# zerr0o/whisper-burn

Measured on AMD Instinct MI355X. Metric: real-time factor (audio-s/wall-s) Whisper Large-V3 Q4 @1/2/4/8 MI355X, higher is better.
Workload: dtype fp16x2

## Files before the change

### include/whisper_amd.h

```cpp
#ifndef WHISPER_AMD_H
#define WHISPER_AMD_H

#include <stddef.h>
#include <stdint.h>

#include "wq4.h"

#ifdef __cplusplus
extern "C" {
#endif

typedef struct wa_model wa_model;

typedef enum wa_variant { WA_LARGE_V3 = 0, WA_MEDIUM = 1, WA_TINY_TEST = 2 } wa_variant;

enum {
  WA_CFG_N_MELS = 0,
  WA_CFG_N_AUDIO_CTX,
  WA_CFG_N_AUDIO_STATE,
  WA_CFG_N_AUDIO_HEAD,
  WA_CFG_N_AUDIO_LAYER,
  WA_CFG_N_TEXT_CTX,
  WA_CFG_N_TEXT_STATE,
  WA_CFG_N_TEXT_HEAD,
  WA_CFG_N_TEXT_LAYER,
  WA_CFG_N_VOCAB,
  WA_CFG_N_LANG,
  WA_CFG_COUNT
};

const char* wa_last_error(void);

wq4_status wa_model_create_synthetic(int device, int variant, uint64_t seed, int max_batch, wq4_precision prec,
                                     wa_model** out);
wq4_status wa_model_create_synthetic_ex(int device, int variant, uint64_t seed, int max_batch, wq4_precision prec,
                                        int weight_type, wa_model** out);
int wa_model_weight_type(const wa_model* m);
int wa_model_wide_range(const wa_model* m);
wq4_status wa_model_create_from_gguf(int device, const char* path, int variant, int max_batch, wq4_precision prec,
                                     wa_model** out);
void wa_model_destroy(wa_model* m);

typedef struct wa_gguf wa_gguf;
wq4_status wa_gguf_open(const char* path, wa_gguf** out);
void wa_gguf_close(wa_gguf* g);
int wa_gguf_version(const wa_gguf* g);
int64_t wa_gguf_tensor_count(const wa_gguf* g);
wq4_status wa_gguf_tensor_info(const wa_gguf* g, int64_t index, char* name, size_t name_cap, int* ndims,
                               uint64_t* dims, int* type, uint64_t* offset, uint64_t* nbytes);
wq4_status wa_gguf_tensor_data(const wa_gguf* g, const char* name, uint8_t* out, size_t cap);
wq4_status wa_model_config(const wa_model* m, int32_t* cfg );
size_t wa_model_device_bytes(const wa_model* m);

wq4_status wa_transcribe(wa_model* m, const float* mel_dev, int n_clips, int lang_token, int max_tokens,
                         int eot_stop, int32_t* tokens_out, int32_t* n_tokens_out, void* stream);

wq4_status wa_transcribe_batches(wa_model* m, const float* mel_dev, int n_batches, int n_clips, int lang_token,
                                 int max_tokens, int eot_stop, int32_t* tokens_out, int32_t* n_tokens_out,
                                 void* stream);
wq4_status wa_last_pipeline_stats(const wa_model* m, float* out );
int wa_last_pipeline_pairs(const wa_model* m);

wq4_status wa_log_mel(int device, const float* audio_dev, int n_clips, int64_t n_samples, int64_t ld_audio,
                      int n_mels, float* mel_dev, void* stream);
wq4_status wa_mel_filterbank(int n_mels, float* filters_out, float* window_out);

wq4_status wa_last_timings(const wa_model* m, float* out );

#define WA_PROF_CATEGORIES 4
wq4_status wa_profile_enable(wa_model* m, int enable);
wq4_status wa_profile_read(wa_model* m, double* out , int reset);

#define WA_PROBE_OUT 6
wq4_status wa_probe_kernels(wa_model* m, int n_clips, int iters, double* out, int out_len);
int wa_decode_group_rows(int n_clips);

wq4_status wa_encode(wa_model* m, const float* mel_dev, int n_clips, float* enc_out_dev, void* stream);
wq4_status wa_prompt_logits(wa_model* m, const int32_t* prompt_dev, int n_clips, int plen, float* logits_dev,
                            void* stream);
wq4_status wa_xattn_check(int device, const float* q_dev, const uint8_t* wk_dev, const uint8_t* wv_dev,
                          const float* bv_dev, int weight_type, const float* enc_dev, int n_clips, int Tq, int T,
                          int H, wq4_precision prec, float* out_dev);
wq4_status wa_xattn_kv_check(int device, const float* q_dev, const float* k_dev, const float* v_dev, int n_clips,
                             int Tq, int T, int H, wq4_precision prec, float* out_dev);

wq4_status wa_transcribe_trace(wa_model* m, const float* mel_dev, int n_clips, int lang_token, int max_tokens,
                               int eot_stop, int32_t* tokens_out, int32_t* n_tokens_out, const int32_t* trace_ids_dev,
                               int trace_k, float* trace_out_dev, void* stream);
wq4_status wa_encoder_attention_check(int device, const float* qkv_dev, int n_clips, int T, int H, wq4_precision prec,
                                      float* out_dev);
wq4_status wa_self_attention_check(int device, const float* qkv_dev, float* cache_k_dev, float* cache_v_dev,
                                   int n_clips, int Tq, int H, int ctx, int kv_len, wq4_precision prec,
                                   float* out_dev);
wq4_status wa_logits_argmax_check(int device, const float* hid_dev, const float* emb_dev, int n_clips, int D, int V,
                                  int step, wq4_precision prec, int32_t* tok_dev, float* logits_dev);
wq4_status wa_synth_uniform(uint64_t seed, const char* name, int64_t n, float lo, float hi, float* out);

#ifdef __cplusplus
}
#endif
#endif
```

### whisper-burn_amd/csrc/whisper/wa_api.cpp

```cpp
#include "wa_model.hpp"

using namespace wa;

namespace {

thread_local std::string g_err;

wq4_status create_model(int device, int variant, int max_batch, wq4_precision prec, int weight_type, Source& src,
                        wa_model** out) {
  WA_HIP(hipSetDevice(device));
  std::unique_ptr<wa_model> m(new wa_model());
  m->device = device;
  m->cfg = preset(variant);
  m->prec = prec;
  m->ns = prec == WQ4_PREC_F16 ? 1 : 2;
  m->bmax = max_batch;
  kv_config(m.get(), max_batch);
  m->wtype = weight_type;
  WA_TRY(build_model(m.get(), src));
  WA_TRY(build_ln_fold(m.get()));
  WA_TRY(alloc_activations(m.get()));
  WA_HIP(hipStreamCreateWithFlags(&m->own_stream, hipStreamNonBlocking));
  WA_HIP(hipDeviceSynchronize());
  *out = m.release();
  return WQ4_OK;
}

}

wq4_status wa::fail(wq4_status s, const std::string& m) {
  g_err = m;
  return s;
}

extern "C" {

const char* wa_last_error(void) { return g_err.c_str(); }

wq4_status wa_model_create_synthetic_ex(int device, int variant, uint64_t seed, int max_batch, wq4_precision prec,
                                        int weight_type, wa_model** out) {
  if (!out) return fail(WQ4_EINVAL, "out is null");
  *out = nullptr;
  if (variant < 0 || variant > 2) return fail(WQ4_EINVAL, "unknown variant");
  if (max_batch < 1 || max_batch > 256) return fail(WQ4_EINVAL, "max_batch must be in [1, 256]");
  if (prec != WQ4_PREC_F16X2 && prec != WQ4_PREC_F16) return fail(WQ4_EINVAL, "unknown precision");
  if (weight_type != 0 && weight_type != 1) return fail(WQ4_EINVAL, "weight_type must be 0 (Q4_0) or 1 (F16)");
  return create_model(device, variant, max_batch, prec, weight_type, *synth_source(seed), out);
}

wq4_status wa_model_create_synthetic(int device, int variant, uint64_t seed, int max_batch, wq4_precision prec,
                                     wa_model** out) {
  return wa_model_create_synthetic_ex(device, variant, seed, max_batch, prec, 0, out);
}

wq4_status wa_model_create_from_gguf(int device, const char* path, int variant, int max_batch, wq4_precision prec,
                                     wa_model** out) {
  if (!out || !path) return fail(WQ4_EINVAL, "null argument");
  *out = nullptr;
  if (variant < 0 || variant > 2) return fail(WQ4_EINVAL, "unknown variant");
  if (max_batch < 1 || max_batch > 256) return fail(WQ4_EINVAL, "max_batch must be in [1, 256]");
  if (prec != WQ4_PREC_F16X2 && prec != WQ4_PREC_F16) return fail(WQ4_EINVAL, "unknown precision");
  GgufFile file;
  if (!file.open(path)) return fail(WQ4_EINVAL, "Failed to parse GGUF: " + file.error());
  const GgufTensor* probe = file.find("encoder.blocks.0.attn.query.weight");
  const int wtype = probe && probe->type == kGgmlF16 ? 1 : 0;
  return create_model(device, variant, max_batch, prec, wtype, *gguf_source(file), out);
}

void wa_model_destroy(wa_model* m) { delete m; }

wq4_status wa_gguf_open(const char* path, wa_gguf** out) {
  if (!path || !out) return fail(WQ4_EINVAL, "null argument");
  *out = nullptr;
  auto* f = new GgufFile();
  if (!f->open(path)) {
    const std::string e = f->error();
    delete f;
    return fail(WQ4_EINVAL, "Failed to parse GGUF: " + e);
  }
  *out = reinterpret_cast<wa_gguf*>(f);
  return WQ4_OK;
}

void wa_gguf_close(wa_gguf* g) { delete reinterpret_cast<GgufFile*>(g); }

int wa_gguf_version(const wa_gguf* g) { return g ? (int)reinterpret_cast<const GgufFile*>(g)->version() : -1; }

int64_t wa_gguf_tensor_count(const wa_gguf* g) {
  return g ? (int64_t)reinterpret_cast<const GgufFile*>(g)->tensors().size() : -1;
}

wq4_status wa_gguf_tensor_info(const wa_gguf* g, int64_t index, char* name, size_t name_cap, int* ndims,
                               uint64_t* dims, int* type, uint64_t* offset, uint64_t* nbytes) {
  if (!g) return fail(WQ4_EINVAL, "null gguf");
  const auto& ts = reinterpret_cast<const GgufFile*>(g)->tensors();
  if (index < 0 || index >= (int64_t)ts.size()) return fail(WQ4_EINVAL, "tensor index out of range");
  const GgufTensor& t = ts[(size_t)index];
  if (name && name_cap) {
    const size_t n = std::min(name_cap - 1, t.name.size());
    std::memcpy(name, t.name.data(), n);
    name[n] = 0;
  }
  if (ndims) *ndims = (int)t.dims.size();
  if (dims)
    for (size_t i = 0; i < t.dims.size(); ++i) dims[i] = t.dims[i];
  if (type) *type = (int)t.type;
  if (offset) *offset = t.offset;
  if (nbytes) *nbytes = t.nbytes();
  return WQ4_OK;
}

wq4_status wa_gguf_tensor_data(const wa_gguf* g, const char* name, uint8_t* out, size_t cap) {
  if (!g || !name || !out) return fail(WQ4_EINVAL, "null argument");
  const auto* f = reinterpret_cast<const GgufFile*>(g);
  const GgufTensor* t = f->find(name);
  if (!t) return fail(WQ4_EINVAL, std::string("Tensor '") + name + "' not found in GGUF");
  const uint8_t* p = f->data(*t);
  if (!p) return fail(WQ4_EINVAL, std::string("Tensor '") + name + "' data lies outside the file");
  if (cap < t->nbytes()) return fail(WQ4_ENOMEM, "output buffer too small");
  std::memcpy(out, p, t->nbytes());
  return WQ4_OK;
}

int wa_model_weight_type(const wa_model* m) { return m ? m->wtype : -1; }

int wa_model_wide_range(const wa_model* m) { return m ? m->range_tier : -1; }

wq4_status wa_model_config(const wa_model* m, int32_t* cfg) {
  if (!m || !cfg) return fail(WQ4_EINVAL, "null argument");
  const Config& c = m->cfg;
  const int32_t v[WA_CFG_COUNT] = {c.n_mels,       c.n_audio_ctx,  c.n_audio_state, c.n_audio_head,
                                   c.n_audio_layer, c.n_text_ctx,   c.n_text_state,  c.n_text_head,
                                   c.n_text_layer,  c.n_vocab,      c.n_lang};
  std::memcpy(cfg, v, sizeof(v));
  return WQ4_OK;
}

size_t wa_model_device_bytes(const wa_model* m) { return m ? m->bytes : 0; }

wq4_status wa_last_timings(const wa_model* m, float* out) {
  if (!m || !out) return fail(WQ4_EINVAL, "null argument");
  std::memcpy(out, m->timings, sizeof(m->timings));
  return WQ4_OK;
}

wq4_status wa_profile_enable(wa_model* m, int enable) {
  if (!m) return fail(WQ4_EINVAL, "null model");
  m->profile = enable != 0;
  return WQ4_OK;
}

wq4_status wa_profile_read(wa_model* m, double* out, int reset) {
  if (!m || !out) return fail(WQ4_EINVAL, "null argument");
  m->resolve_profile();
  std::memcpy(out, m->prof, sizeof(m->prof));
  if (reset) std::memset(m->prof, 0, sizeof(m->prof));
  return WQ4_OK;
}

wq4_status wa_encode(wa_model* m, const float* mel_dev, int n_clips, float* enc_out_dev, void* stream) {
  if (!m || !mel_dev) return fail(WQ4_EINVAL, "null argument");
  if (n_clips < 1 || n_clips > m->bmax) return fail(WQ4_EINVAL, "n_clips out of range");
  WA_HIP(hipSetDevice(m->device));
  hipStream_t st = static_cast<hipStream_t>(stream);
  WA_TRY(encoder_forward(m, mel_dev, n_clips, st, enc_out_dev));
  return cross_kv_forward(m, n_clips, st, false);
}

wq4_status wa_prompt_logits(wa_model* m, const int32_t* prompt_dev, int n_clips, int plen, float* logits_dev,
                            void* stream) {
  if (!m || !prompt_dev || !logits_dev) return fail(WQ4_EINVAL, "null argument");
  if (n_clips < 1 || n_clips > m->bmax || plen < 1 || plen > 4) return fail(WQ4_EINVAL, "bad n_clips / plen");
  if (n_clips > m->kv_batch) return fail(WQ4_EINVAL, "wa_encode the clips first");
  WA_HIP(hipSetDevice(m->device));
  hipStream_t st = static_cast<hipStream_t>(stream);
  DecGroup& g = m->groups[0];
  g.lane = 0;
  g.b0 = 0;
  g.nb = n_clips;
  WA_TRY(decoder_forward(m, g, prompt_dev, plen, nullptr, 0, 0, st));
  WA_HIP(hipMemcpyAsync(logits_dev, g.logits, (size_t)n_clips * m->cfg.n_vocab * 4, hipMemcpyDeviceToDevice, st));
  return WQ4_OK;
}

int wa_decode_group_rows(int n_clips) {
  if (n_clips < 1) return 0;
  const int G = decode_groups(n_clips);
  return (n_clips + G - 1) / G;
}

constexpr int kProbeOut = WA_PROBE_OUT;

wq4_status wa_probe_kernels(wa_model* m, int n_clips, int iters, double* out, int out_len) {
  if (!m || !out) return fail(WQ4_EINVAL, "null argument");
  if (out_len < kProbeOut) return fail(WQ4_EINVAL, "out holds fewer than 6 doubles");
  if (n_clips < 1 || n_clips > m->bmax || iters < 1) return fail(WQ4_EINVAL, "bad n_clips / iters");
  if (n_clips > m->kv_batch) return fail(WQ4_EINVAL, "run wa_transcribe / wa_encode on n_clips clips first");
  WA_HIP(hipSetDevice(m->device));
  hipStream_t st = m->own_stream;
  const Config& c = m->cfg;
  const int B = n_clips, D = c.n_text_state, T = c.n_audio_ctx, H = c.n_text_head;
  DecLayer& L = m->dec[0];
  DecGroup g = m->groups[0];
  const _Float16* enc = m->enc_planes;
  hipEvent_t a, b;
  WA_HIP(hipEventCreate(&a));
  WA_HIP(hipEventCreate(&b));
  float ms = 0.0f;
  g.b0 = 0;
  g.nb = B;
  const bool kv = m->group_kv(g);
  auto xattn = [&]() -> hipError_t {
    if (kv)
      return launch_cross_attention_kv(g.qd, L.xk, L.xv, B, 1, T, H, g.xkv_part, g.xkv_ctr, g.atd_dec, m->ns, st);
    return launch_xattn(g.qd, L.ck_raw, L.cv_raw, L.cv_p, L.cv_b, m->wtype, enc, B, 1, T, H, D, g.xqt, g.xattn_part,
                        g.atd_dec, m->ns, st);
  };
  WA_HIP(xattn());
  WA_HIP(hipEventRecord(a, st));
  for (int i = 0; i < iters; ++i) WA_HIP(xattn());
  WA_HIP(hipEventRecord(b, st));
  WA_HIP(hipEventSynchronize(b));
  WA_HIP(hipEventElapsedTime(&ms, a, b));
  out[0] = ms * 1e3 / iters;
  const double wbytes = m->wtype == 1 ? 2.0 * D * D * 2 : 2.0 * D * D * 18 / 32;
  out[1] = kv ? (double)B * T * D * 4 * 2 + (double)B * D * (4 + 2 * m->ns)
              : (double)B * T * D * 2 * m->ns + wbytes + (double)B * D * (4 + 2 * m->ns);
  out[5] = kv ? 1.0 : 0.0;
  const int F = 4 * D;
  WA_WQ4(wq4_gemm_tiled(L.fc1, L.fc1_b, g.atd_dec, nullptr, nullptr, g.atf_dec, B, WQ4_EPI_GELU | WQ4_EPI_TILED_OUT,
                        m->prec, 2, st));
  WA_HIP(hipEventRecord(a, st));
  for (int i = 0; i < iters; ++i)
    WA_WQ4(wq4_gemm_tiled(L.fc1, L.fc1_b, g.atd_dec, nullptr, nullptr, g.atf_dec, B,
                          WQ4_EPI_GELU | WQ4_EPI_TILED_OUT, m->prec, 2, st));
  WA_HIP(hipEventRecord(b, st));
  WA_HIP(hipEventSynchronize(b));
  WA_HIP(hipEventElapsedTime(&ms, a, b));
  out[2] = ms * 1e3 / iters;
  out[3] = (double)F * D * 18 / 32 + (double)B * D * 2 * m->ns + (double)B * F * 2 * m->ns;
  out[4] = 2.0 * B * F * D;
  (void)hipEventDestroy(a);
  (void)hipEventDestroy(b);
  return WQ4_OK;
}

}
```

### whisper-burn_amd/csrc/whisper/wa_checks.cpp

```cpp
#include <map>
#include <mutex>

#include "wa_mel.hpp"
#include "wa_model.hpp"

using namespace wa;

namespace {

int planes(wq4_precision prec) { return prec == WQ4_PREC_F16 ? 1 : 2; }

template <class Launch>
wq4_status tiled_check(Dev& d, int64_t R, int D, wq4_precision prec, float* out_dev, Launch launch) {
  const size_t tb = wq4_atiled_bytes(R, D, prec);
  auto* tiled = d.alloc<_Float16>(tb / 2);
  if (!tiled) return fail(WQ4_ENOMEM, "allocation failed");
  WA_HIP(hipMemset(tiled, 0, tb));
  WA_HIP(launch(tiled));
  WA_HIP(launch_untile(tiled, (int)R, D, planes(prec), out_dev, nullptr));
  WA_HIP(hipDeviceSynchronize());
  return WQ4_OK;
}

}

extern "C" {

wq4_status wa_xattn_check(int device, const float* q_dev, const uint8_t* wk_dev, const uint8_t* wv_dev,
                          const float* bv_dev, int weight_type, const float* enc_dev, int n_clips, int Tq, int T,
                          int H, wq4_precision prec, float* out_dev) {
  if (!q_dev || !wk_dev || !wv_dev || !bv_dev || !enc_dev || !out_dev) return fail(WQ4_EINVAL, "null argument");
  if (n_clips < 1 || Tq < 1 || T < 1 || H < 1) return fail(WQ4_EINVAL, "bad sizes");
  const int D = 64 * H, ns = planes(prec), R = n_clips * Tq;
  const int HP = (H + 15) / 16 * 16;
  WA_HIP(hipSetDevice(device));
  Dev d;
  auto* enc = d.alloc<_Float16>((size_t)n_clips * T * ns * D);
  auto* qt = d.alloc<_Float16>((size_t)R * ns * HP * D);
  auto* part = d.alloc<float>(xattn_part_floats(R, H, D, T));
  if (!enc || !qt || !part) return fail(WQ4_ENOMEM, "allocation failed");
  WA_HIP(hipMemset(qt, 0, (size_t)R * ns * HP * D * 2));
  WA_HIP(launch_enc_planes(enc_dev, (int64_t)n_clips * T, D, ns, enc, nullptr));
  uint32_t* wvp = nullptr;
  if (weight_type == 0) {
    wvp = d.alloc<uint32_t>(wv_pack_words(H, D));
    if (!wvp) return fail(WQ4_ENOMEM, "allocation failed");
    WA_HIP(launch_wv_pack(wv_dev, H, D, wvp, nullptr));
  }
  return tiled_check(d, R, D, prec, out_dev, [&](_Float16* tiled) {
    return launch_xattn(q_dev, wk_dev, wv_dev, wvp, bv_dev, weight_type, enc, n_clips, Tq, T, H, D, qt, part, tiled,
                        ns, nullptr);
  });
}

wq4_status wa_xattn_kv_check(int device, const float* q_dev, const float* k_dev, const float* v_dev, int n_clips,
                             int Tq, int T, int H, wq4_precision prec, float* out_dev) {
  if (!q_dev || !k_dev || !v_dev || !out_dev) return fail(WQ4_EINVAL, "null argument");
  if (n_clips < 1 || Tq < 1 || Tq > 4 || T < 1 || H < 1) return fail(WQ4_EINVAL, "bad sizes");
  WA_HIP(hipSetDevice(device));
  Dev d;
  auto* part = d.alloc<float>(cross_attention_kv_part_floats(n_clips, H, T));
  auto* ctr = d.alloc<int>((size_t)n_clips * H);
  if (!part || !ctr) return fail(WQ4_ENOMEM, "allocation failed");
  WA_HIP(hipMemset(ctr, 0, (size_t)n_clips * H * sizeof(int)));
  return tiled_check(d, n_clips * Tq, 64 * H, prec, out_dev, [&](_Float16* tiled) {
    return launch_cross_attention_kv(q_dev, k_dev, v_dev, n_clips, Tq, T, H, part, ctr, tiled, planes(prec), nullptr);
  });
}

wq4_status wa_encoder_attention_check(int device, const float* qkv_dev, int n_clips, int T, int H, wq4_precision prec,
                                      float* out_dev) {
  if (!qkv_dev || !out_dev) return fail(WQ4_EINVAL, "null argument");
  if (n_clips < 1 || T < 1 || H < 1) return fail(WQ4_EINVAL, "bad sizes");
  WA_HIP(hipSetDevice(device));
  Dev d;
  return tiled_check(d, (int64_t)n_clips * T, 64 * H, prec, out_dev, [&](_Float16* tiled) {
    return launch_encoder_attention(qkv_dev, n_clips, T, H, tiled, planes(prec), nullptr);
  });
}

wq4_status wa_self_attention_check(int device, const float* qkv_dev, float* cache_k_dev, float* cache_v_dev,
                                   int n_clips, int Tq, int H, int ctx, int kv_len, wq4_precision prec,
                                   float* out_dev) {
  if (!qkv_dev || !cache_k_dev || !cache_v_dev || !out_dev) return fail(WQ4_EINVAL, "null argument");
  if (n_clips < 1 || Tq < 1 || Tq > 4 || H < 1 || ctx < 1 || ctx > 448 || kv_len < 0 || kv_len + Tq > ctx)
    return fail(WQ4_EINVAL, "bad sizes");
  WA_HIP(hipSetDevice(device));
  Dev d;
  return tiled_check(d, n_clips * Tq, 64 * H, prec, out_dev, [&](_Float16* tiled) {
    return launch_decoder_self_attention(qkv_dev, cache_k_dev, cache_v_dev, n_clips, Tq, H, ctx, nullptr, kv_len,
                                         tiled, planes(prec), nullptr);
  });
}

wq4_status wa_logits_argmax_check(int device, const float* hid_dev, const float* emb_dev, int n_clips, int D, int V,
                                  int step, wq4_precision prec, int32_t* tok_dev, float* logits_dev) {
  if (!hid_dev || !emb_dev || !tok_dev) return fail(WQ4_EINVAL, "null argument");
  if (n_clips < 1 || n_clips > 32 || V < 1 || !emb_tiled_supported(D)) return fail(WQ4_EINVAL, "bad sizes");
  const int ns = planes(prec);
  WA_HIP(hipSetDevice(device));
  Dev d;
  const int64_t erows = emb_tiled_rows(V);
  const int ng = logits_argmax_groups(V);
  auto* emb2 = d.alloc<_Float16>((size_t)erows * ns * D);
  auto* st = d.alloc<DecodeState>(1);
  auto* pval = d.alloc<float>((size_t)32 * ng);
  auto* pidx = d.alloc<int>((size_t)32 * ng);
  auto* ctr = d.alloc<int>(1);
  const size_t tb = wq4_atiled_bytes(n_clips, D, prec);
  auto* ht = d.alloc<_Float16>(tb / 2);
  int* ids = nullptr;
  if (logits_dev) ids = d.alloc<int>((size_t)n_clips * 2 * V);
  if (!emb2 || !st || !pval || !pidx || !ctr || !ht || (logits_dev && !ids))
    return fail(WQ4_ENOMEM, "allocation failed");
  WA_HIP(launch_emb_tiled(emb_dev, V, D, ns, emb2, nullptr));
  WA_WQ4(wq4_tile_activations(hid_dev, n_clips, D, D, prec, ht, tb, nullptr));
  const DecodeState s0{0, 0, logits_dev ? 0 : step, 0};
  const int min_tokens = !logits_dev ? kMinTokens : (step + 1 < kMinTokens ? 1 << 30 : 0);
  WA_HIP(hipMemcpy(st, &s0, sizeof(s0), hipMemcpyHostToDevice));
  WA_HIP(hipMemset(ctr, 0, sizeof(int)));
  float* tr = nullptr;
  if (logits_dev) {
    std::vector<int> h((size_t)n_clips * 2 * V, 0);
    for (int b = 0; b < n_clips; ++b)
      for (int v = 0; v < V; ++v) h[((size_t)b * 2 + 1) * V + v] = v;
    WA_HIP(hipMemcpy(ids, h.data(), h.size() * 4, hipMemcpyHostToDevice));
    tr = d.alloc<float>((size_t)n_clips * 2 * V);
    if (!tr) return fail(WQ4_ENOMEM, "allocation failed");
  }
  WA_HIP(launch_logits_argmax(ht, n_clips, D, emb2, ns, V, min_tokens, st, pval, pidx, ctr, tok_dev, ids, tr, 2, V,
                              nullptr, nullptr));
  if (logits_dev)
    for (int b = 0; b < n_clips; ++b)
      WA_HIP(hipMemcpy(logits_dev + (size_t)b * V, tr + ((size_t)b * 2 + 1) * V, (size_t)V * 4,
                       hipMemcpyDeviceToDevice));
  WA_HIP(hipDeviceSynchronize());
  return WQ4_OK;
}

}

namespace {
struct MelDevice {
  std::map<int, uint8_t*> consts;
  float* part = nullptr;
  int part_clips = 0;
};
std::mutex g_mel_mu;
std::map<int, MelDevice> g_mel;
}

extern "C" {

wq4_status wa_log_mel(int device, const float* audio_dev, int n_clips, int64_t n_samples, int64_t ld_audio,
                      int n_mels, float* mel_dev, void* stream) {
  if (!mel_dev || (!audio_dev && n_samples > 0)) return fail(WQ4_EINVAL, "null argument");
  if (n_clips < 1) return fail(WQ4_EINVAL, "n_clips must be >= 1");
  if (n_samples < 0 || ld_audio < n_samples) return fail(WQ4_EINVAL, "need 0 <= n_samples <= ld_audio");
  if (n_mels < 1 || n_mels > kMelMaxMels) return fail(WQ4_EINVAL, "n_mels must be in [1, 256]");
  WA_HIP(hipSetDevice(device));
  hipStream_t st = static_cast<hipStream_t>(stream);
  std::lock_guard<std::mutex> lk(g_mel_mu);
  MelDevice& md = g_mel[device];
  uint8_t*& c = md.consts[n_mels];
  if (!c || md.part_clips < n_clips) {
    hipStreamCaptureStatus cs = hipStreamCaptureStatusNone;
    WA_HIP(hipStreamIsCapturing(st, &cs));
    if (cs != hipStreamCaptureStatusNone)
      return fail(WQ4_EINVAL, "wa_log_mel: run once outside stream capture first (allocates constants)");
  }
  if (!c) {
    const MelBank bank = make_mel_bank(n_mels);
    std::vector<uint8_t> host(mel_const_bytes(n_mels));
    mel_pack_consts(bank, host.data());
    WA_HIP(hipMalloc(reinterpret_cast<void**>(&c), host.size()));
    WA_HIP(hipMemcpy(c, host.data(), host.size(), hipMemcpyHostToDevice));
  }
  if (md.part_clips < n_clips) {
    WA_HIP(hipDeviceSynchronize());
    if (md.part) WA_HIP(hipFree(md.part));
    md.part = nullptr;
    md.part_clips = 0;
    WA_HIP(hipMalloc(reinterpret_cast<void**>(&md.part), (size_t)n_clips * kMelWgPerClip * sizeof(float)));
    md.part_clips = n_clips;
  }
  WA_HIP(launch_log_mel(audio_dev, n_clips, n_samples, ld_audio, n_mels, c, md.part, mel_dev, st));
  return WQ4_OK;
}

wq4_status wa_mel_filterbank(int n_mels, float* filters_out, float* window_out) {
  if (n_mels < 1 || n_mels > kMelMaxMels) return fail(WQ4_EINVAL, "n_mels must be in [1, 256]");
  const MelBank bank = make_mel_bank(n_mels);
  if (filters_out) std::memcpy(filters_out, bank.filters.data(), bank.filters.size() * sizeof(float));
  if (window_out) std::memcpy(window_out, bank.window.data(), bank.window.size() * sizeof(float));
  return WQ4_OK;
}

}
```

### whisper-burn_amd/csrc/whisper/wa_forward.cpp

```cpp
#include "wa_model.hpp"

using namespace wa;

namespace {

constexpr int kSOT = 50258;

struct Prof {
  wa_model* m;
  hipStream_t st;
  int cat;
  double gflop, gb;
  hipEvent_t a = nullptr, b = nullptr;
  Prof(wa_model* m_, hipStream_t st_, int cat_, double gflop_, double gb_)
      : m(m_), st(st_), cat(cat_), gflop(gflop_), gb(gb_) {
    if (m->profile && st != m->enc_stream && hipEventCreate(&a) == hipSuccess && hipEventCreate(&b) == hipSuccess)
      (void)hipEventRecord(a, st);
  }
  ~Prof() {
    if (a && b) {
      (void)hipEventRecord(b, st);
      m->pending.push_back({a, b, cat, gflop, gb});
    }
  }
};

Prof q4prof(wa_model* m, hipStream_t st, const wq4_tensor* w, int64_t rows) {
  int64_t n = 0, k = 0;
  (void)wq4_tensor_shape(w, &n, &k);
  return Prof(m, st, 0, 2.0 * rows * n * k * 1e-9, ((double)n * k * 18 / 32 + 4.0 * rows * k + 4.0 * rows * n) * 1e-9);
}

bool lnfold_on(const wa_model* m, int Tq, const DecodeState* state, int64_t rows) {
  static const bool enabled = [] {
    const char* e = getenv("WA_LN_FOLD");
    return e ? atoi(e) != 0 : true;
  }();
  if (!enabled || !m->fold_allowed() || state == nullptr || Tq != 1 || m->dec.empty()) return false;
  const DecLayer& L = m->dec[0];
  for (const wq4_tensor* w : {L.qkv, L.out, L.cq, L.cout, L.fc1, L.fc2})
    if (!wq4_lnfold_supported(w, rows)) return false;
  return true;
}

bool fused_pick(const DecGroup& g, int Tq, const DecodeState* state) {
  return state != nullptr && Tq == 1 && g.nb <= 32;
}

wq4_status decode_step(wa_model* m, DecGroup& g, int eot_stop, hipStream_t st) {
  WA_HIP(launch_bookkeep(g.next_tok, g.tokens, g.ntok, g.done, g.nb, kMaxTokens, eot_stop, g.state, st));
  WA_TRY(decoder_forward(m, g, g.next_tok, 1, g.state, 0, 0, st));
  if (!fused_pick(g, 1, g.state))
    WA_HIP(launch_argmax_step(g.logits, g.nb, m->cfg.n_vocab, kMinTokens, g.state, g.next_tok, m->range_flag, st));
  return WQ4_OK;
}

}

namespace wa {

wq4_status alloc_activations(wa_model* m) {
  const Config& c = m->cfg;
  const int D = c.n_audio_state, F = 4 * D, Dt = c.n_text_state, Ft = 4 * Dt;
  const int B = m->bmax, T = c.n_audio_ctx;
  const int64_t renc = (int64_t)B * T, rdec = (int64_t)B * 4;
  Dev& d = m->dev;
  auto tiled = [&](int64_t rows, int k) {
    const size_t n = wq4_atiled_bytes(rows, k, m->prec);
    m->bytes += n;
    return d.alloc<_Float16>(n / 2);
  };
  auto f32 = [&](int64_t n) {
    m->bytes += (size_t)n * 4;
    return d.alloc<float>((size_t)n);
  };
  m->h1 = f32((int64_t)B * 2 * T * D);
  m->x = f32(renc * D);
  m->qkv = f32(renc * 3 * D);
  m->at_d = tiled(renc, D);
  m->at_f = tiled(renc, F);
  m->enc_planes = d.alloc<_Float16>((size_t)renc * m->ns * D);
  m->bytes += (size_t)renc * m->ns * D * 2;
  for (auto& L : m->dec) {
    L.cache_k = f32((int64_t)B * c.n_text_ctx * Dt);
    L.cache_v = f32((int64_t)B * c.n_text_ctx * Dt);
  }
  if (!emb_tiled_supported(Dt)) return fail(WQ4_EINVAL, "n_text_state must be a multiple of 128");
  const size_t erows = (size_t)emb_tiled_rows(c.n_vocab);
  m->tok_emb2 = d.alloc<_Float16>(erows * m->ns * Dt);
  if (!m->tok_emb2) return fail(WQ4_ENOMEM, "embedding plane allocation failed");
  m->bytes += erows * m->ns * Dt * 2;
  WA_HIP(launch_emb_tiled(m->tok_emb, c.n_vocab, Dt, m->ns, m->tok_emb2, nullptr));
  const int HP = (c.n_text_head + 15) / 16 * 16;
  size_t xpart = 0;
  for (int r = 1; r <= rdec; ++r) xpart = std::max(xpart, xattn_part_floats(r, c.n_text_head, Dt, T));
  m->groups.resize(kMaxGroups);
  for (DecGroup& g : m->groups) {
    g.xd = f32(rdec * Dt);
    g.qkvd = f32(rdec * 3 * Dt);
    g.qd = f32(rdec * Dt);
    g.hid = f32(rdec * Dt);
    g.logits = f32((int64_t)B * c.n_vocab);
    g.atd_dec = tiled(rdec, Dt);
    g.atf_dec = tiled(rdec, Ft);
    g.prompt_tok = d.alloc<int>(rdec);
    g.next_tok = d.alloc<int>(B);
    g.tokens = d.alloc<int>((size_t)B * kMaxTokens);
    g.ntok = d.alloc<int>(B);
    g.done = d.alloc<int>(B);
    g.state = d.alloc<DecodeState>(1);
    g.xattn_part = f32((int64_t)xpart);
    const int kvc = std::max(1, m->kv_clips);
    g.xkv_part = f32((int64_t)cross_attention_kv_part_floats(kvc, c.n_text_head, T));
    g.xkv_ctr = d.alloc<int>((size_t)kvc * c.n_text_head);
    g.xqt = d.alloc<_Float16>((size_t)rdec * m->ns * HP * Dt);
    g.atd_ln = tiled(rdec, Dt);
    g.ln_stats = f32(rdec * (Dt / 16) * 2);
    g.hid_t = tiled(rdec, Dt);
    g.lg_val = f32((int64_t)32 * logits_argmax_groups(c.n_vocab));
    g.lg_idx = d.alloc<int>((size_t)32 * logits_argmax_groups(c.n_vocab));
    g.lg_ctr = d.alloc<int>(1);
    m->bytes += (size_t)rdec * m->ns * HP * Dt * 2;
    for (void* p : {(void*)g.xd, (void*)g.qkvd, (void*)g.qd, (void*)g.hid, (void*)g.logits, (void*)g.atd_dec,
                    (void*)g.atf_dec, (void*)g.prompt_tok, (void*)g.next_tok, (void*)g.tokens, (void*)g.ntok,
                    (void*)g.done, (void*)g.state, (void*)g.xattn_part, (void*)g.xqt, (void*)g.lg_val,
                    (void*)g.lg_idx, (void*)g.lg_ctr, (void*)g.atd_ln, (void*)g.ln_stats, (void*)g.hid_t,
                    (void*)g.xkv_part, (void*)g.xkv_ctr})
      if (!p) return fail(WQ4_ENOMEM, "decode-group allocation failed");
    WA_HIP(hipMemset(g.xkv_ctr, 0, (size_t)kvc * c.n_text_head * sizeof(int)));
    WA_HIP(hipMemset(g.atd_ln, 0, wq4_atiled_bytes(rdec, Dt, m->prec)));
    WA_HIP(hipMemset(g.hid_t, 0, wq4_atiled_bytes(rdec, Dt, m->prec)));
    WA_HIP(hipMemset(g.lg_ctr, 0, sizeof(int)));
    WA_HIP(hipMemset(g.xqt, 0, (size_t)rdec * m->ns * HP * Dt * 2));
    WA_HIP(hipMemset(g.atd_dec, 0, wq4_atiled_bytes(rdec, Dt, m->prec)));
    WA_HIP(hipMemset(g.atf_dec, 0, wq4_atiled_bytes(rdec, Ft, m->prec)));
    WA_HIP(hipHostMalloc(reinterpret_cast<void**>(&g.host_ndone), 8 * sizeof(int), 0));
    WA_HIP(hipStreamCreateWithFlags(&g.st, hipStreamNonBlocking));
  }
  m->range_flag = d.alloc<int>(1);
  for (void* p : {(void*)m->h1, (void*)m->x, (void*)m->qkv, (void*)m->at_d, (void*)m->at_f, (void*)m->enc_planes,
                  (void*)m->range_flag})
    if (!p) return fail(WQ4_ENOMEM, "activation allocation failed");
  WA_HIP(hipMemset(m->range_flag, 0, sizeof(int)));
  for (auto& L : m->dec)
    if (!L.cache_k || !L.cache_v) return fail(WQ4_ENOMEM, "KV cache allocation failed");
  WA_HIP(hipMemset(m->at_d, 0, wq4_atiled_bytes(renc, D, m->prec)));
  WA_HIP(hipMemset(m->at_f, 0, wq4_atiled_bytes(renc, F, m->prec)));
  return WQ4_OK;
}

wq4_status encoder_front(wa_model* m, const float* mel, int B, hipStream_t st) {
  const Config& c = m->cfg;
  const int D = c.n_audio_state, T = c.n_audio_ctx;
  const int T_mel = 2 * T;
  const int64_t rows = (int64_t)B * T;
  {
    Prof p(m, st, 2, 2.0 * B * T_mel * D * 3.0 * c.n_mels * 1e-9, 4.0 * B * T_mel * (c.n_mels + D) * 1e-9);
    WA_HIP(launch_conv_gelu(mel, (long)c.n_mels * T_mel, T_mel, 1, B, c.n_mels, T_mel, 1, m->conv1_wt, m->conv1_b,
                            nullptr, D, m->h1, st));
  }
  {
    Prof p(m, st, 2, 2.0 * rows * D * 3.0 * D * 1e-9, 4.0 * B * (T_mel + T) * D * 1e-9);
    WA_HIP(launch_conv_gelu(m->h1, (long)T_mel * D, 1, D, B, D, T_mel, 2, m->conv2_wt, m->conv2_b, m->enc_pos, D,
                            m->x, st));
  }
  return WQ4_OK;
}

wq4_status encoder_layers(wa_model* m, int B, int l0, int l1, hipStream_t st) {
  const Config& c = m->cfg;
  const int D = c.n_audio_state, T = c.n_audio_ctx, H = c.n_audio_head;
  const int64_t rows = (int64_t)B * T;
  const double ln_gb = 8.0 * rows * D * 1e-9;
  for (int li = l0; li < l1; ++li) {
    const EncLayer& L = m->enc[li];
    {
      Prof p(m, st, 3, 0.0, ln_gb);
      WA_WQ4(wq4_layernorm(m->x, L.ln1_w, L.ln1_b, rows, D, m->prec, m->at_d, nullptr, st));
    }
    {
      Prof p = q4prof(m, st, L.qkv, rows);
      WA_WQ4(wq4_gemm_tiled(L.qkv, L.qkv_b, m->at_d, nullptr, m->qkv, nullptr, rows, 0u, m->prec, 1, st));
    }
    {
      Prof p(m, st, 1, 4.0 * B * H * (double)T * T * 64 * 1e-9, 16.0 * rows * D * 1e-9);
      WA_HIP(launch_encoder_attention(m->qkv, B, T, H, m->at_d, m->ns, st, m->f32_attn() ? m->h1 : nullptr));
    }
    if (m->f32_attn()) {
      WA_WQ4(wq4_linear_forward_ws(L.out, L.out_b, m->h1, m->x, m->x, rows, D, WQ4_EPI_RESIDUAL, m->prec, m->at_d,
                                   wq4_atiled_bytes(rows, D, m->prec), st));
    } else {
      Prof p = q4prof(m, st, L.out, rows);
      WA_WQ4(wq4_gemm_tiled(L.out, L.out_b, m->at_d, m->x, m->x, nullptr, rows, WQ4_EPI_RESIDUAL, m->prec, 1, st));
    }
    if (m->abi_ffn()) {
      WA_WQ4(wq4_layernorm(m->x, L.ln2_w, L.ln2_b, rows, D, WQ4_PREC_F16X2, nullptr, m->qkv, st));
      WA_WQ4(wq4_ffn_forward_ws(L.fc1, L.fc1_b, L.fc2, L.fc2_b, m->qkv, m->x, m->x, rows, WQ4_EPI_RESIDUAL, m->prec,
                                m->ffn_ws, m->ffn_ws_bytes, st));
      continue;
    }
    {
      Prof p(m, st, 3, 0.0, ln_gb);
      WA_WQ4(wq4_layernorm(m->x, L.ln2_w, L.ln2_b, rows, D, m->prec, m->at_d, nullptr, st));
    }
    {
      Prof p = q4prof(m, st, L.fc1, rows);
      WA_WQ4(wq4_gemm_tiled(L.fc1, L.fc1_b, m->at_d, nullptr, nullptr, m->at_f, rows,
                            WQ4_EPI_GELU | WQ4_EPI_TILED_OUT, m->prec, 1, st));
    }
    {
      Prof p = q4prof(m, st, L.fc2, rows);
      WA_WQ4(wq4_gemm_tiled(L.fc2, L.fc2_b, m->at_f, m->x, m->x, nullptr, rows, WQ4_EPI_RESIDUAL, m->prec, 1, st));
    }
  }
  return WQ4_OK;
}

wq4_status encoder_post(wa_model* m, int B, hipStream_t st, float* enc_out_f32) {
  const Config& c = m->cfg;
  const int D = c.n_audio_state;
  const int64_t rows = (int64_t)B * c.n_audio_ctx;
  Prof p(m, st, 3, 0.0, 8.0 * rows * D * 1e-9);
  float* out = enc_out_f32 ? enc_out_f32 : m->h1;
  WA_WQ4(wq4_layernorm(m->x, m->lnp_w, m->lnp_b, rows, D, WQ4_PREC_F16X2, nullptr, out, st));
  m->enc_f32 = out;
  return WQ4_OK;
}

wq4_status encoder_forward(wa_model* m, const float* mel, int B, hipStream_t st, float* enc_out_f32) {
  WA_TRY(encoder_front(m, mel, B, st));
  WA_TRY(encoder_layers(m, B, 0, (int)m->enc.size(), st));
  return encoder_post(m, B, st, enc_out_f32);
}

wq4_status cross_kv_forward(wa_model* m, int B, hipStream_t st, bool caches, int lane) {
  const Config& c = m->cfg;
  const int64_t rows = (int64_t)B * c.n_audio_ctx;
  if (lane == 1) {
    WA_HIP(launch_enc_planes(m->enc_f32, rows, c.n_audio_state, m->ns, m->enc_planes2, st));
    return WQ4_OK;
  }
  m->kv_batch = B;
  WA_HIP(launch_enc_planes(m->enc_f32, rows, c.n_audio_state, m->ns, m->enc_planes, st));
  m->kv_n = caches && B <= m->kv_small ? B : 0;
  if (m->kv_n > 0 && !m->kv_alloc_ok) {
    const size_t n = (size_t)m->kv_clips * c.n_audio_ctx * c.n_text_state;
    bool ok = true;
    for (DecLayer& L : m->dec) {
      if (!L.xk) L.xk = m->dev.alloc<float>(n);
      if (!L.xv) L.xv = m->dev.alloc<float>(n);
      if (!L.xk || !L.xv) {
        ok = false;
        break;
      }
    }
    if (!ok) {
      for (DecLayer& L : m->dec) {
        m->dev.release(L.xk);
        m->dev.release(L.xv);
        L.xk = L.xv = nullptr;
      }
      m->kv_n = 0;
      return fail(WQ4_ENOMEM, "cross K/V cache allocation failed");
    }
    m->bytes += n * 8 * m->dec.size();
    m->kv_alloc_ok = true;
  }
  if (m->kv_n > 0) {
    const int64_t kv_rows = (int64_t)m->kv_n * c.n_audio_ctx;
    WA_WQ4(wq4_layernorm(m->x, m->lnp_w, m->lnp_b, kv_rows, c.n_audio_state, m->prec, m->at_d, nullptr, st));
    for (DecLayer& L : m->dec) {
      WA_WQ4(wq4_gemm_tiled_headmajor(L.ck, nullptr, m->at_d, L.xk, kv_rows, c.n_audio_ctx, c.n_text_state, m->prec,
                                      0, st));
      WA_WQ4(wq4_gemm_tiled_headmajor(L.cv, L.cv_b, m->at_d, L.xv, kv_rows, c.n_audio_ctx, c.n_text_state, m->prec,
                                      0, st));
    }
  }
  return WQ4_OK;
}

wq4_status decoder_forward(wa_model* m, DecGroup& g, const int* tokens, int Tq, const DecodeState* state, int pos0,
                           int kv0, hipStream_t st) {
  const Config& c = m->cfg;
  const int D = c.n_text_state, H = c.n_text_head, T = c.n_audio_ctx;
  const int B = g.nb;
  const int64_t rows = (int64_t)B * Tq;
  const size_t self_ofs = (size_t)g.b0 * H * c.n_text_ctx * 64;
  const _Float16* enc = (g.lane ? m->enc_planes2 : m->enc_planes) + (size_t)g.b0 * T * m->ns * c.n_audio_state;
  const bool fold = lnfold_on(m, Tq, state, rows);
  float* const a32 = m->f32_attn() ? g.hid : nullptr;
  auto ln_gemm = [&](const wq4_tensor* w, const float* bias, const float* wg, const float* b2, const float* lw,
                     const float* lb, float* y, void* yt, unsigned flags) -> wq4_status {
    if (fold) {
      const wq4_ln_fold cons{nullptr, nullptr, nullptr, g.ln_stats, wg};
      WA_WQ4(wq4_gemm_tiled_lnfold(w, b2, g.atd_ln, nullptr, y, yt, rows, flags, m->prec, &cons, st));
    } else {
      WA_WQ4(wq4_layernorm(g.xd, lw, lb, rows, D, m->prec, g.atd_dec, nullptr, st));
      WA_WQ4(wq4_gemm_tiled(w, bias, g.atd_dec, nullptr, y, yt, rows, flags, m->prec, 2, st));
    }
    return WQ4_OK;
  };
  auto resid_gemm = [&](const wq4_tensor* w, const float* bias, const void* at, const float* x32,
                        const float* next_lw) -> wq4_status {
    if (x32) {
      WA_WQ4(wq4_linear_forward_ws(w, bias, x32, g.xd, g.xd, rows, D, WQ4_EPI_RESIDUAL, m->prec, g.atd_dec,
                                   wq4_atiled_bytes(rows, D, m->prec), st));
    } else if (fold) {
      const wq4_ln_fold prod{next_lw, next_lw ? g.atd_ln : nullptr, next_lw ? g.ln_stats : nullptr, nullptr, nullptr};
      WA_WQ4(wq4_gemm_tiled_lnfold(w, bias, at, g.xd, g.xd, nullptr, rows, WQ4_EPI_RESIDUAL, m->prec, &prod, st));
    } else {
      WA_WQ4(wq4_gemm_tiled(w, bias, at, g.xd, g.xd, nullptr, rows, WQ4_EPI_RESIDUAL, m->prec, 2, st));
    }
    return WQ4_OK;
  };
  if (fold)
    WA_HIP(launch_embed_fold(tokens, m->tok_emb, m->dec_pos, B, Tq, D, state, pos0, g.xd, m->dec[0].ln1_w, g.atd_ln,
                             g.ln_stats, m->ns, st));
  else
    WA_HIP(launch_embed(tokens, m->tok_emb, m->dec_pos, B, Tq, D, state, pos0, g.xd, st));
  const int nl = (int)m->dec.size();
  for (int li = 0; li < nl; ++li) {
    DecLayer& L = m->dec[li];
    WA_TRY(ln_gemm(L.qkv, L.qkv_b, L.qkv_wg, L.qkv_b2, L.ln1_w, L.ln1_b, g.qkvd, nullptr, 0u));
    WA_HIP(launch_decoder_self_attention(g.qkvd, (g.lane ? L.cache_k2 : L.cache_k) + self_ofs,
                                         (g.lane ? L.cache_v2 : L.cache_v) + self_ofs, B, Tq, H, c.n_text_ctx, state,
                                         kv0, g.atd_dec, m->ns, st, a32));
    WA_TRY(resid_gemm(L.out, L.out_b, g.atd_dec, a32, L.ln2_w));
    WA_TRY(ln_gemm(L.cq, L.cq_b, L.cq_wg, L.cq_b2, L.ln2_w, L.ln2_b, g.qd, nullptr, 0u));
    if (m->group_kv(g)) {
      const size_t kofs = (size_t)g.b0 * T * D;
      WA_HIP(launch_cross_attention_kv(g.qd, L.xk + kofs, L.xv + kofs, B, Tq, T, H, g.xkv_part, g.xkv_ctr, g.atd_dec,
                                       m->ns, st, a32));
    } else {
      WA_HIP(launch_xattn(g.qd, L.ck_raw, L.cv_raw, L.cv_p, L.cv_b, m->wtype, enc, B, Tq, T, H, D, g.xqt,
                          g.xattn_part, g.atd_dec, m->ns, st, a32));
    }
    WA_TRY(resid_gemm(L.cout, L.cout_b, g.atd_dec, a32, L.ln3_w));
    if (m->abi_ffn()) {
      WA_WQ4(wq4_layernorm(g.xd, L.ln3_w, L.ln3_b, rows, D, WQ4_PREC_F16X2, nullptr, g.hid, st));
      WA_WQ4(wq4_ffn_forward_ws(L.fc1, L.fc1_b, L.fc2, L.fc2_b, g.hid, g.xd, g.xd, rows, WQ4_EPI_RESIDUAL, m->prec,
                                g.ffn_ws, g.ffn_ws_bytes, st));
      continue;
    }
    WA_TRY(ln_gemm(L.fc1, L.fc1_b, L.fc1_wg, L.fc1_b2, L.ln3_w, L.ln3_b, nullptr, g.atf_dec,
                   WQ4_EPI_GELU | WQ4_EPI_TILED_OUT));
    WA_TRY(resid_gemm(L.fc2, L.fc2_b, g.atf_dec, nullptr, li + 1 < nl ? m->dec[li + 1].ln1_w : nullptr));
  }
  if (fused_pick(g, Tq, state)) {
    WA_WQ4(wq4_layernorm(g.xd, m->dln_w, m->dln_b, rows, D, m->prec, g.hid_t, nullptr, st));
    const size_t tofs = (size_t)g.b0 * m->trace_s1 * m->trace_k;
    WA_HIP(launch_logits_argmax(g.hid_t, B, D, m->tok_emb2, m->ns, c.n_vocab, kMinTokens, state, g.lg_val, g.lg_idx,
                                g.lg_ctr, g.next_tok, m->trace_out ? m->trace_ids + tofs : nullptr,
                                m->trace_out ? m->trace_out + tofs : nullptr, m->trace_s1, m->trace_k, m->range_flag,
                                st));
    return WQ4_OK;
  }
  WA_WQ4(wq4_layernorm(g.xd, m->dln_w, m->dln_b, rows, D, WQ4_PREC_F16X2, nullptr, g.hid, st));
  WA_HIP(launch_logits(g.hid + (size_t)(Tq - 1) * D, B, D, (int64_t)Tq * D, m->tok_emb, c.n_vocab, g.logits, st));
  return WQ4_OK;
}

wq4_status prompt_group(wa_model* m, DecGroup& g, int lang_token, hipStream_t st) {
  const Config& c = m->cfg;
  const int B = g.nb;
  std::vector<int> ptok((size_t)B * 4);
  int pos0, kv0;
  if (lang_token >= 0) {
    for (int b = 0; b < B; ++b) {
      ptok[b * 4 + 0] = kSOT;
      ptok[b * 4 + 1] = lang_token;
      ptok[b * 4 + 2] = c.transcribe_token();
      ptok[b * 4 + 3] = c.no_timestamps_token();
    }
    WA_HIP(hipMemcpyAsync(g.prompt_tok, ptok.data(), (size_t)B * 4 * 4, hipMemcpyHostToDevice, st));
    WA_TRY(decoder_forward(m, g, g.prompt_tok, 4, nullptr, 0, 0, st));
    pos0 = 4;
    kv0 = 4;
  } else {
    for (int b = 0; b < B; ++b) {
      ptok[b * 3 + 0] = kSOT;
      ptok[b * 3 + 1] = c.transcribe_token();
      ptok[b * 3 + 2] = c.no_timestamps_token();
    }
    WA_HIP(hipMemcpyAsync(g.prompt_tok, ptok.data(), (size_t)B * 3 * 4, hipMemcpyHostToDevice, st));
    std::vector<int> sot(B, kSOT);
    WA_HIP(hipMemcpyAsync(g.next_tok, sot.data(), (size_t)B * 4, hipMemcpyHostToDevice, st));
    WA_TRY(decoder_forward(m, g, g.next_tok, 1, nullptr, 0, 0, st));
    WA_HIP(launch_argmax(g.logits, B, c.n_vocab, 50259, 50259 + c.n_lang, 0, nullptr, g.prompt_tok, 3, m->range_flag,
                         st));
    WA_TRY(decoder_forward(m, g, g.prompt_tok, 3, nullptr, 0, 0, st));
    pos0 = 4;
    kv0 = 3;
  }
  WA_HIP(launch_argmax(g.logits, B, c.n_vocab, 0, c.n_vocab, 1, nullptr, g.next_tok, 1, m->range_flag, st));
  const DecodeState init{pos0 - 1, kv0 - 1, -1, 0};
  WA_HIP(hipMemcpyAsync(g.state, &init, sizeof(init), hipMemcpyHostToDevice, st));
  WA_HIP(hipMemsetAsync(g.ntok, 0, (size_t)B * 4, st));
  WA_HIP(hipMemsetAsync(g.done, 0, (size_t)B * 4, st));
  WA_HIP(hipMemsetAsync(g.tokens, 0, (size_t)B * kMaxTokens * 4, st));
  return WQ4_OK;
}

wq4_status ensure_graph(wa_model* m, DecGroup& g, int eot_stop) {
  const int64_t key =
      ((((((int64_t)g.lane * 512 + g.b0) * 512 + g.nb) * 2 + (eot_stop ? 1 : 0)) * 2 + (m->trace_out ? 1 : 0)) * 2 +
       (m->group_kv(g) ? 1 : 0)) * 4 + m->range_tier;
  if (g.graph && g.graph_key == key) return WQ4_OK;
  std::swap(g.graph, g.graph_alt);
  std::swap(g.graph_key, g.graph_alt_key);
  if (g.graph && g.graph_key == key) return WQ4_OK;
  if (g.graph) {
    (void)hipGraphExecDestroy(g.graph);
    g.graph = nullptr;
  }
  WA_WQ4(wq4_prepare_stream(m->device, g.st));
  hipGraph_t gr;
  WA_HIP(hipStreamBeginCapture(g.st, hipStreamCaptureModeThreadLocal));
  wq4_status s = decode_step(m, g, eot_stop, g.st);
  hipError_t ce = hipStreamEndCapture(g.st, &gr);
  if (s != WQ4_OK) return s;
  if (ce != hipSuccess) return fail(WQ4_EHIP, std::string("graph capture: ") + hipGetErrorString(ce));
  ce = hipGraphInstantiate(&g.graph, gr, nullptr, nullptr, 0);
  (void)hipGraphDestroy(gr);
  if (ce != hipSuccess) return fail(WQ4_EHIP, std::string("graph instantiate: ") + hipGetErrorString(ce));
  g.graph_key = key;
  return WQ4_OK;
}

void kv_config(wa_model* m, int max_batch) {
  static const int small = [] {
    const char* e = getenv("WA_XATTN_KV_CLIPS");
    return e ? std::max(0, atoi(e)) : 8;
  }();
  m->kv_small = std::min(small, max_batch);
  m->kv_clips = m->kv_small;
}

wq4_status ensure_ffn_ws(wa_model* m) {
  if (m->ffn_ws) return WQ4_OK;
  const DecLayer& Ld = m->dec.front();
  const EncLayer& Le = m->enc.front();
  const size_t ne = wq4_ffn_workspace_bytes(Le.fc1, Le.fc2, (int64_t)m->bmax * m->cfg.n_audio_ctx);
  const size_t nd = wq4_ffn_workspace_bytes(Ld.fc1, Ld.fc2, (int64_t)m->bmax * 4);
  if (ne == 0 || nd == 0) return fail(WQ4_EINVAL, "FFN workspace size");
  void* e = m->dev.alloc<uint8_t>(ne);
  bool ok = e != nullptr;
  for (DecGroup& g : m->groups) {
    g.ffn_ws = ok ? m->dev.alloc<uint8_t>(nd) : nullptr;
    ok = ok && g.ffn_ws != nullptr;
  }
  if (!ok) {
    m->dev.release(e);
    for (DecGroup& g : m->groups) {
      m->dev.release(g.ffn_ws);
      g.ffn_ws = nullptr;
      g.ffn_ws_bytes = 0;
    }
    return fail(WQ4_ENOMEM, "range tier 2: FFN workspace allocation failed");
  }
  for (DecGroup& g : m->groups) {
    g.ffn_ws_bytes = nd;
    m->bytes += nd;
  }
  m->ffn_ws = e;
  m->ffn_ws_bytes = ne;
  m->bytes += ne;
  return WQ4_OK;
}

bool ensure_pair_lane(wa_model* m) {
  if (m->enc_planes2) return true;
  const Config& c = m->cfg;
  const size_t np = (size_t)m->bmax * c.n_audio_ctx * m->ns * c.n_audio_state;
  const size_t nc = (size_t)m->bmax * c.n_text_ctx * c.n_text_state;
  _Float16* planes = m->dev.alloc<_Float16>(np);
  bool ok = planes != nullptr;
  for (DecLayer& L : m->dec) {
    if (!ok) break;
    L.cache_k2 = m->dev.alloc<float>(nc);
    L.cache_v2 = m->dev.alloc<float>(nc);
    ok = L.cache_k2 && L.cache_v2;
  }
  if (!ok) {
    (void)hipGetLastError();
    m->dev.release(planes);
    for (DecLayer& L : m->dec) {
      m->dev.release(L.cache_k2);
      m->dev.release(L.cache_v2);
      L.cache_k2 = L.cache_v2 = nullptr;
    }
    return false;
  }
  m->enc_planes2 = planes;
  m->bytes += np * 2 + nc * 8 * m->dec.size();
  return true;
}

int decode_groups(int B) {
  static const int forced = [] {
    const char* env = getenv("WA_DECODE_GROUPS");
    return env ? atoi(env) : 0;
  }();
  int G = forced > 0 ? forced : (B >= 16 ? 2 : 1);
  if (G > kMaxGroups) G = kMaxGroups;
  if (G > B) G = B;
  return G;
}

}
```

### whisper-burn_amd/csrc/whisper/wa_kernels.hpp

```cpp
#pragma once
#include <hip/hip_runtime_api.h>
#include <stdint.h>

namespace wa {

struct DecodeState {
  int position;
  int kv_len;
  int step;
  int n_done;
};

hipError_t launch_encoder_attention(const float* qkv, int B, int T, int H, _Float16* tiled, int ns,
                                    hipStream_t st, float* out32 = nullptr);

hipError_t launch_decoder_self_attention(const float* qkv, float* cache_k, float* cache_v, int B, int Tq, int H,
                                         int ctx, const DecodeState* state, int kv_len_host, _Float16* tiled,
                                         int ns, hipStream_t st, float* out32 = nullptr);

int cross_attention_kv_splits(int T);
size_t cross_attention_kv_part_floats(int B, int H, int T);
hipError_t launch_cross_attention_kv(const float* q, const float* k, const float* v, int B, int Tq, int T, int H,
                                     float* part, int* counters, _Float16* tiled, int ns, hipStream_t st,
                                     float* out32 = nullptr);

struct XattnPlan {
  int splits;
  int ch;
};
XattnPlan xattn_plan(int R, int T);
size_t xattn_part_floats(int R, int H, int D, int T);
size_t wv_pack_words(int H, int D);
hipError_t launch_wv_pack(const uint8_t* wv, int H, int D, uint32_t* out, hipStream_t st);
hipError_t launch_xattn(const float* q, const uint8_t* wk, const uint8_t* wv, const uint32_t* wvp, const float* bv,
                        int wtype, const _Float16* enc, int B, int Tq, int T, int H, int D, _Float16* qt, float* part,
                        _Float16* tiled, int ns, hipStream_t st, float* out32 = nullptr);
hipError_t launch_untile(const _Float16* tiled, int R, int K, int ns, float* out, hipStream_t st);
hipError_t launch_enc_planes(const float* x, int64_t rows, int D, int ns, _Float16* out, hipStream_t st);

hipError_t launch_conv_gelu(const float* in, long in_bs, long in_cs, long in_ts, int B, int C, int T_in,
                            int stride, const float* w_t, const float* bias, const float* pos, int N, float* out,
                            hipStream_t st);

hipError_t launch_embed(const int* tokens, const float* tok_emb, const float* pos_emb, int B, int Tq, int D,
                        const DecodeState* state, int pos0_host, float* x, hipStream_t st);

hipError_t launch_embed_fold(const int* tokens, const float* tok_emb, const float* pos_emb, int B, int Tq, int D,
                             const DecodeState* state, int pos0_host, float* x, const float* gamma, _Float16* at,
                             float* stats, int ns, hipStream_t st);

hipError_t launch_logits(const float* h, int B, int D, long ldh, const float* emb, int V, float* logits,
                         hipStream_t st);

hipError_t launch_argmax(const float* logits, int B, int V, int lo, int hi, int suppress_eot,
                         const DecodeState* state, int* out_tok, int out_stride, int* range_flag, hipStream_t st);

int logits_argmax_groups(int V);
hipError_t launch_logits_argmax(const _Float16* htiled, int B, int D, const _Float16* emb2, int ns, int V,
                                int min_tokens, const DecodeState* state, float* pval, int* pidx, int* counter,
                                int* out_tok, const int* trace_ids, float* trace_out, int trace_s1, int trace_k,
                                int* range_flag, hipStream_t st);
bool emb_tiled_supported(int D);
int64_t emb_tiled_rows(int V);
hipError_t launch_emb_tiled(const float* emb, int V, int D, int ns, _Float16* out, hipStream_t st);

hipError_t launch_bookkeep(const int* next_tok, int* tokens, int* n_tokens, int* done, int B, int max_tokens,
                           int eot_stop, DecodeState* state, hipStream_t st);

hipError_t launch_argmax_step(const float* logits, int B, int V, int min_tokens, const DecodeState* state,
                              int* out_tok, int* range_flag, hipStream_t st);

}
```

### whisper-burn_amd/csrc/whisper/wa_model.hpp

```cpp
#pragma once
#include <hip/hip_runtime_api.h>

#include <algorithm>
#include <cstring>
#include <memory>
#include <string>
#include <vector>

#include "../../../include/whisper_amd.h"
#include "../../../include/wq4.h"
#include "wa_gguf.hpp"
#include "wa_kernels.hpp"

namespace wa {

wq4_status fail(wq4_status s, const std::string& m);

#define WA_HIP(expr)                                                                                \
  do {                                                                                              \
    hipError_t e_ = (expr);                                                                         \
    if (e_ != hipSuccess) return wa::fail(WQ4_EHIP, std::string(#expr) + ": " + hipGetErrorString(e_)); \
  } while (0)
#define WA_WQ4(expr)                                                                    \
  do {                                                                                  \
    wq4_status s_ = (expr);                                                             \
    if (s_ != WQ4_OK) return wa::fail(s_, std::string(#expr) + ": " + wq4_last_error()); \
  } while (0)
#define WA_TRY(expr)             \
  do {                           \
    wq4_status s_ = (expr);      \
    if (s_ != WQ4_OK) return s_; \
  } while (0)

constexpr int kMaxTokens = 224;
constexpr int kMinTokens = 3;

struct Config {
  int n_mels, n_audio_ctx, n_audio_state, n_audio_head, n_audio_layer;
  int n_text_ctx, n_text_state, n_text_head, n_text_layer, n_vocab, n_lang;
  int transcribe_token() const { return 50260 + n_lang; }
  int no_timestamps_token() const { return transcribe_token() + 4; }
};

struct Dev {
  std::vector<void*> ptrs;
  ~Dev() {
    for (void* p : ptrs) (void)hipFree(p);
  }
  template <class T>
  T* alloc(size_t n) {
    void* p = nullptr;
    if (hipMalloc(&p, n * sizeof(T) + 256) != hipSuccess) return nullptr;
    ptrs.push_back(p);
    return static_cast<T*>(p);
  }
  void release(void* p) {
    if (!p) return;
    for (void*& q : ptrs)
      if (q == p) {
        (void)hipFree(q);
        q = ptrs.back();
        ptrs.pop_back();
        return;
      }
  }
};

struct EncLayer {
  float *ln1_w, *ln1_b, *ln2_w, *ln2_b, *qkv_b, *out_b, *fc1_b, *fc2_b;
  wq4_tensor *qkv = nullptr, *out = nullptr, *fc1 = nullptr, *fc2 = nullptr;
};
struct DecLayer {
  float *ln1_w, *ln1_b, *ln2_w, *ln2_b, *ln3_w, *ln3_b;
  float *qkv_b, *out_b, *cq_b, *cv_b, *cout_b, *fc1_b, *fc2_b;
  wq4_tensor *qkv = nullptr, *out = nullptr, *cq = nullptr, *cout = nullptr, *fc1 = nullptr, *fc2 = nullptr;
  float *qkv_wg = nullptr, *qkv_b2 = nullptr, *cq_wg = nullptr, *cq_b2 = nullptr, *fc1_wg = nullptr,
        *fc1_b2 = nullptr;
  uint8_t *ck_raw = nullptr, *cv_raw = nullptr;
  uint32_t* cv_p = nullptr;
  float *cache_k, *cache_v;
  float *cache_k2 = nullptr, *cache_v2 = nullptr;
  wq4_tensor *ck = nullptr, *cv = nullptr;
  float *xk = nullptr, *xv = nullptr;
};

constexpr int kMaxGroups = 4;
struct DecGroup {
  hipStream_t st = nullptr;
  int b0 = 0, nb = 0;
  int lane = 0;
  float *xd, *qkvd, *qd, *hid, *logits;
  _Float16 *atd_dec, *atf_dec;
  int *prompt_tok, *next_tok, *tokens, *ntok, *done;
  _Float16* xqt;
  float* xattn_part;
  float* xkv_part;
  int* xkv_ctr;
  _Float16* atd_ln;
  float* ln_stats;
  _Float16* hid_t;
  float* lg_val;
  int *lg_idx, *lg_ctr;
  DecodeState* state;
  void* ffn_ws = nullptr;
  size_t ffn_ws_bytes = 0;
  int* host_ndone = nullptr;
  hipGraphExec_t graph = nullptr;
  int64_t graph_key = -1;
  hipGraphExec_t graph_alt = nullptr;
  int64_t graph_alt_key = -1;
};

}

struct wa_model {
  int device = 0;
  wa::Config cfg{};
  wq4_precision prec = WQ4_PREC_F16X2;
  int ns = 2;
  int bmax = 1;
  wa::Dev dev;
  size_t bytes = 0;
  float *conv1_wt, *conv1_b, *conv2_wt, *conv2_b, *enc_pos, *lnp_w, *lnp_b;
  float *tok_emb, *dec_pos, *dln_w, *dln_b;
  _Float16* tok_emb2 = nullptr;
  std::vector<wa::EncLayer> enc;
  std::vector<wa::DecLayer> dec;
  float *h1, *x, *qkv;
  _Float16 *at_d, *at_f;
  _Float16* enc_planes = nullptr;
  _Float16* enc_planes2 = nullptr;
  const float* enc_f32 = nullptr;
  std::vector<wa::DecGroup> groups;
  int wtype = 0;
  int kv_batch = 0;
  int kv_clips = 0, kv_small = 0;
  int kv_n = 0;
  bool kv_alloc_ok = false;
  bool group_kv(const wa::DecGroup& g) const { return g.nb > 0 && g.b0 + g.nb <= kv_n; }
  hipStream_t own_stream = nullptr;
  hipStream_t enc_stream = nullptr;
  int enc_cus = 0;
  int overlap_k = -1;
  int overlap_b = 0, overlap_eot = -1;
  float pipe[4] = {0, 0, 0, 0};
  int pipe_pairs = 0;
  int* range_flag = nullptr;
  int range_tier = 0;
  bool fold_allowed() const { return range_tier < 1; }
  bool abi_ffn() const { return range_tier >= 2; }
  bool f32_attn() const { return range_tier >= 3; }
  void* ffn_ws = nullptr;
  size_t ffn_ws_bytes = 0;
  float timings[5] = {0, 0, 0, 0, 0};
  const int* trace_ids = nullptr;
  float* trace_out = nullptr;
  int trace_s1 = 0, trace_k = 0;
  struct Pending {
    hipEvent_t a, b;
    int cat;
    double gflop, gb;
  };
  bool profile = false;
  std::vector<Pending> pending;
  double prof[WA_PROF_CATEGORIES][4] = {};

  void resolve_profile() {
    for (auto& p : pending) {
      float ms = 0.0f;
      if (hipEventSynchronize(p.b) == hipSuccess && hipEventElapsedTime(&ms, p.a, p.b) == hipSuccess) {
        prof[p.cat][0] += 1;
        prof[p.cat][1] += ms;
        prof[p.cat][2] += p.gflop;
        prof[p.cat][3] += p.gb;
      }
      (void)hipEventDestroy(p.a);
      (void)hipEventDestroy(p.b);
    }
    pending.clear();
  }

  ~wa_model() {
    resolve_profile();
    for (auto& g : groups) {
      if (g.graph) (void)hipGraphExecDestroy(g.graph);
      if (g.graph_alt) (void)hipGraphExecDestroy(g.graph_alt);
      if (g.st) (void)hipStreamDestroy(g.st);
      if (g.host_ndone) (void)hipHostFree(g.host_ndone);
    }
    if (own_stream) (void)hipStreamDestroy(own_stream);
    if (enc_stream) (void)hipStreamDestroy(enc_stream);
    for (auto& l : enc)
      for (wq4_tensor* t : {l.qkv, l.out, l.fc1, l.fc2}) wq4_tensor_destroy(t);
    for (auto& l : dec)
      for (wq4_tensor* t : {l.qkv, l.out, l.cq, l.cout, l.fc1, l.fc2, l.ck, l.cv}) wq4_tensor_destroy(t);
  }
};

namespace wa {

Config preset(int variant);
struct Source {
  virtual ~Source() = default;
  virtual bool f32(const std::string& name, int64_t n, float lo, float hi, bool optional, std::vector<float>& out) = 0;
  virtual bool linear(const std::string& name, int rows, int k, int wtype, uint8_t* dst) = 0;
  std::string err;
};
std::unique_ptr<Source> synth_source(uint64_t seed);
std::unique_ptr<Source> gguf_source(const GgufFile& f);
wq4_status build_model(wa_model* m, Source& src);
wq4_status build_ln_fold(wa_model* m);

void kv_config(wa_model* m, int max_batch);
wq4_status alloc_activations(wa_model* m);
wq4_status ensure_ffn_ws(wa_model* m);
int decode_groups(int B);
wq4_status encoder_front(wa_model* m, const float* mel, int B, hipStream_t st);
wq4_status encoder_layers(wa_model* m, int B, int l0, int l1, hipStream_t st);
wq4_status encoder_post(wa_model* m, int B, hipStream_t st, float* enc_out_f32);
wq4_status encoder_forward(wa_model* m, const float* mel, int B, hipStream_t st, float* enc_out_f32);
wq4_status cross_kv_forward(wa_model* m, int B, hipStream_t st, bool caches, int lane = 0);
bool ensure_pair_lane(wa_model* m);
wq4_status decoder_forward(wa_model* m, DecGroup& g, const int* tokens, int Tq, const DecodeState* state, int pos0,
                           int kv0, hipStream_t st);
wq4_status prompt_group(wa_model* m, DecGroup& g, int lang_token, hipStream_t st);
wq4_status ensure_graph(wa_model* m, DecGroup& g, int eot_stop);

}
```

### whisper-burn_amd/csrc/whisper/wa_transcribe.cpp

```cpp
#include "wa_model.hpp"

using namespace wa;

namespace {

constexpr int kEncOverlapCUs = 32;
constexpr int kEncOverlapLayers0 = 16;
constexpr double kEncOverlapFill = 0.98;

struct EventSet {
  std::vector<hipEvent_t> e;
  EventSet() = default;
  EventSet(const EventSet&) = delete;
  EventSet& operator=(const EventSet&) = delete;
  ~EventSet() {
    for (hipEvent_t x : e) (void)hipEventDestroy(x);
  }
  hipError_t make(hipEvent_t* out, bool timing = true) {
    hipError_t r = hipEventCreateWithFlags(out, timing ? hipEventDefault : hipEventDisableTiming);
    if (r == hipSuccess) e.push_back(*out);
    return r;
  }
};

constexpr int kPairMinClips = 16, kPairMaxClips = 32;

bool pair_enabled() {
  static const bool enabled = [] {
    const char* e = getenv("WA_PAIR_BATCHES");
    return e ? atoi(e) != 0 : true;
  }();
  return enabled;
}

int unit_groups(int B, bool pair) { return pair ? 2 : decode_groups(B); }

wq4_status run_decode(wa_model* m, int B, bool pair, int lang_token, int max_tokens, int eot_stop, hipEvent_t ready,
                      const hipEvent_t* gprompt, const hipEvent_t* gdone, int* gsteps) {
  const int G = unit_groups(B, pair);
  for (int i = 0; i < G; ++i) {
    DecGroup& g = m->groups[i];
    g.lane = pair ? i : 0;
    g.b0 = pair ? 0 : (int)((int64_t)B * i / G);
    g.nb = pair ? B : (int)((int64_t)B * (i + 1) / G) - g.b0;
    WA_HIP(hipStreamWaitEvent(g.st, ready, 0));
    WA_TRY(prompt_group(m, g, lang_token, g.st));
    WA_HIP(hipEventRecord(gprompt[i], g.st));
    WA_TRY(ensure_graph(m, g, eot_stop));
  }
  EventSet ev;
  hipEvent_t ring[kMaxGroups][8];
  if (eot_stop)
    for (int i = 0; i < G; ++i)
      for (auto& e : ring[i]) WA_HIP(ev.make(&e, false));
  const int lag = 4;
  bool live[kMaxGroups] = {};
  int nlive = G;
  for (int i = 0; i < G; ++i) {
    live[i] = true;
    gsteps[i] = 0;
  }
  for (int step = 0; step < max_tokens && nlive > 0; ++step) {
    for (int i = 0; i < G; ++i) {
      if (!live[i]) continue;
      DecGroup& g = m->groups[i];
      WA_HIP(hipGraphLaunch(g.graph, g.st));
      ++gsteps[i];
      if (eot_stop) {
        const int slot = step % 8;
        WA_HIP(hipMemcpyAsync(&g.host_ndone[slot], &g.state->n_done, sizeof(int), hipMemcpyDeviceToHost, g.st));
        WA_HIP(hipEventRecord(ring[i][slot], g.st));
      }
    }
    if (eot_stop && step >= lag) {
      const int old = (step - lag) % 8;
      for (int i = 0; i < G; ++i) {
        if (!live[i]) continue;
        WA_HIP(hipEventSynchronize(ring[i][old]));
        if (m->groups[i].host_ndone[old] >= m->groups[i].nb) {
          live[i] = false;
          --nlive;
        }
      }
    }
  }
  for (int i = 0; i < G; ++i) WA_HIP(hipEventRecord(gdone[i], m->groups[i].st));
  return WQ4_OK;
}

wq4_status collect_batch(wa_model* m, int B, bool pair, const hipEvent_t* gdone, hipStream_t st, int32_t* tok,
                         int32_t* nt, int* flag, size_t lane_stride) {
  const int G = unit_groups(B, pair);
  for (int i = 0; i < G; ++i) WA_HIP(hipStreamWaitEvent(st, gdone[i], 0));
  for (int i = 0; i < G; ++i) {
    const DecGroup& g = m->groups[i];
    const size_t ofs = g.lane * lane_stride;
    WA_HIP(hipMemcpyAsync(tok + ofs + (size_t)g.b0 * kMaxTokens, g.tokens, (size_t)g.nb * kMaxTokens * 4,
                          hipMemcpyDeviceToHost, st));
    WA_HIP(hipMemcpyAsync(nt + ofs + g.b0, g.ntok, (size_t)g.nb * 4, hipMemcpyDeviceToHost, st));
  }
  for (int i = 0; i < (pair ? 2 : 1); ++i)
    WA_HIP(hipMemcpyAsync(flag + i * lane_stride, m->range_flag, sizeof(int), hipMemcpyDeviceToHost, st));
  return WQ4_OK;
}

void copy_tokens(const int32_t* tok, const int32_t* nt, int B, int max_tokens, int32_t* tokens_out,
                 int32_t* n_tokens_out) {
  for (int b = 0; b < B; ++b) {
    n_tokens_out[b] = std::min(nt[b], max_tokens);
    std::memcpy(tokens_out + (size_t)b * max_tokens, tok + (size_t)b * kMaxTokens, (size_t)max_tokens * 4);
  }
}

wq4_status transcribe_once(wa_model* m, const float* mel_dev, int n_clips, int lang_token, int max_tokens,
                           int eot_stop, int32_t* tokens_out, int32_t* n_tokens_out, void* stream, bool* overflow) {
  hipStream_t st = m->own_stream;
  const int B = n_clips;
  const int G = decode_groups(B);
  EventSet ev;
  hipEvent_t e_in, e_enc, e_kv, e_ready, e_end, gprompt[kMaxGroups], gdone[kMaxGroups];
  for (hipEvent_t* e : {&e_in, &e_enc, &e_kv, &e_ready, &e_end}) WA_HIP(ev.make(e));
  for (int i = 0; i < G; ++i) {
    WA_HIP(ev.make(&gprompt[i]));
    WA_HIP(ev.make(&gdone[i]));
  }
  WA_HIP(hipEventRecord(e_in, static_cast<hipStream_t>(stream)));
  WA_HIP(hipStreamWaitEvent(st, e_in, 0));
  WA_HIP(hipMemsetAsync(m->range_flag, 0, sizeof(int), st));

  WA_HIP(hipEventRecord(e_enc, st));
  WA_TRY(encoder_forward(m, mel_dev, B, st, nullptr));
  WA_HIP(hipEventRecord(e_kv, st));
  WA_TRY(cross_kv_forward(m, B, st, true));
  WA_HIP(hipEventRecord(e_ready, st));
  int gsteps[kMaxGroups] = {};
  WA_TRY(run_decode(m, B, false, lang_token, max_tokens, eot_stop, e_ready, gprompt, gdone, gsteps));
  const int steps = *std::max_element(gsteps, gsteps + G);
  std::vector<int32_t> tok((size_t)B * kMaxTokens), nt(B);
  int flag = 0;
  WA_TRY(collect_batch(m, B, false, gdone, st, tok.data(), nt.data(), &flag, 0));
  WA_HIP(hipEventRecord(e_end, st));
  WA_HIP(hipStreamSynchronize(st));
  *overflow = flag != 0;
  copy_tokens(tok.data(), nt.data(), B, max_tokens, tokens_out, n_tokens_out);
  float t_enc = 0.0f, t_kv = 0.0f, tp = 0.0f, tall = 0.0f;
  WA_HIP(hipEventElapsedTime(&t_enc, e_enc, e_kv));
  WA_HIP(hipEventElapsedTime(&t_kv, e_kv, e_ready));
  for (int i = 0; i < G; ++i) {
    float t = 0.0f;
    WA_HIP(hipEventElapsedTime(&t, e_ready, gprompt[i]));
    tp = std::max(tp, t);
  }
  WA_HIP(hipEventElapsedTime(&tall, e_ready, e_end));
  m->timings[0] = t_enc;
  m->timings[1] = t_kv;
  m->timings[2] = tp;
  m->timings[3] = tall - tp;
  m->timings[4] = (float)steps;
  return WQ4_OK;
}

wq4_status ensure_enc_stream(wa_model* m) {
  if (m->enc_stream) return WQ4_OK;
  hipDeviceProp_t prop;
  WA_HIP(hipGetDeviceProperties(&prop, m->device));
  const int total = prop.multiProcessorCount;
  int n = kEncOverlapCUs;
  if (const char* e = getenv("WA_ENC_CUS")) n = atoi(e);
  n = std::max(8, std::min(total, n));
  std::vector<uint32_t> mask((total + 31) / 32, 0u);
  for (int i = 0; i < n; ++i) mask[i / 32] |= 1u << (i % 32);
  WA_HIP(hipExtStreamCreateWithCUMask(&m->enc_stream, (uint32_t)mask.size(), mask.data()));
  m->enc_cus = n;
  return WQ4_OK;
}

wq4_status transcribe_pipelined(wa_model* m, const float* mel_dev, int NB, int B, int lang_token, int max_tokens,
                                int eot_stop, int32_t* tokens_out, int32_t* n_tokens_out, void* stream, int* flags) {
  WA_TRY(ensure_enc_stream(m));
  hipStream_t st = m->own_stream, es = m->enc_stream;
  const int L = (int)m->enc.size();
  const size_t mel_stride = (size_t)B * m->cfg.n_mels * 2 * m->cfg.n_audio_ctx;
  const bool pairing = pair_enabled() && NB >= 2 && B >= kPairMinClips && B <= kPairMaxClips && B > m->kv_small &&
                       decode_groups(B) == 2 && ensure_pair_lane(m);
  int32_t* host = nullptr;
  const size_t per = (size_t)B * kMaxTokens + B + 1;
  WA_HIP(hipHostMalloc(reinterpret_cast<void**>(&host), (size_t)NB * per * 4, 0));
  struct HostGuard {
    wa_model* m;
    int32_t* p;
    bool done = false;
    ~HostGuard() {
      if (!done) {
        (void)hipStreamSynchronize(m->own_stream);
        if (m->enc_stream) (void)hipStreamSynchronize(m->enc_stream);
        for (DecGroup& g : m->groups)
          if (g.st) (void)hipStreamSynchronize(g.st);
      }
      (void)hipHostFree(p);
    }
  } hg{m, host};
  EventSet ev;
  struct Unit {
    int first = 0, n = 1;
    hipEvent_t ready, mstart, mend, pstart, gprompt[kMaxGroups], gdone[kMaxGroups];
    int k = 0, gsteps[kMaxGroups] = {};
  };
  std::vector<Unit> ut;
  for (int i = 0; i < NB; i += ut.back().n) {
    ut.emplace_back();
    ut.back().first = i;
    ut.back().n = pairing && NB - i >= 2 ? 2 : 1;
  }
  const int NU = (int)ut.size();
  for (Unit& u : ut) {
    for (hipEvent_t* e : {&u.ready, &u.mstart, &u.mend, &u.pstart}) WA_HIP(ev.make(e));
    for (int i = 0; i < unit_groups(B, u.n == 2); ++i) {
      WA_HIP(ev.make(&u.gprompt[i]));
      WA_HIP(ev.make(&u.gdone[i]));
    }
  }
  auto unit_encoder = [&](Unit& u, int k0) -> wq4_status {
    for (int j = 0; j < u.n; ++j) {
      if (j == 0 && k0 >= 0) {
        WA_TRY(encoder_layers(m, B, k0, L, st));
        WA_TRY(encoder_post(m, B, st, nullptr));
      } else {
        WA_TRY(encoder_forward(m, mel_dev + (u.first + j) * mel_stride, B, st, nullptr));
      }
      WA_TRY(cross_kv_forward(m, B, st, true, j));
    }
    WA_HIP(hipMemsetAsync(m->range_flag, 0, sizeof(int), st));
    WA_HIP(hipEventRecord(u.ready, st));
    return WQ4_OK;
  };
  hipEvent_t e_in, e_enc0;
  WA_HIP(ev.make(&e_in));
  WA_HIP(ev.make(&e_enc0));
  WA_HIP(hipEventRecord(e_in, static_cast<hipStream_t>(stream)));
  WA_HIP(hipStreamWaitEvent(st, e_in, 0));
  WA_HIP(hipEventRecord(e_enc0, st));
  WA_TRY(unit_encoder(ut[0], -1));
  if (m->overlap_k < 0 || m->overlap_b != B || m->overlap_eot != eot_stop) m->overlap_k = std::min(L, kEncOverlapLayers0);
  m->overlap_b = B;
  m->overlap_eot = eot_stop;
  double t_exposed = 0.0, t_masked = 0.0, t_decode = 0.0, t_prompt = 0.0, k_sum = 0.0;
  int32_t steps_all = 0;
  for (int i = 0; i < NU; ++i) {
    Unit& u = ut[i];
    const bool pair = u.n == 2;
    if (i >= 1) {
      Unit& p = ut[i - 1];
      const int PG = unit_groups(B, p.n == 2);
      for (int g = 0; g < PG; ++g) WA_HIP(hipEventSynchronize(p.gdone[g]));
      WA_HIP(hipEventSynchronize(p.mend));
      float td = 0.0f, tm = 0.0f;
      for (int g = 0; g < PG; ++g) {
        float t = 0.0f;
        WA_HIP(hipEventElapsedTime(&t, p.ready, p.gdone[g]));
        td = std::max(td, t);
      }
      WA_HIP(hipEventElapsedTime(&tm, p.mstart, p.mend));
      if (!getenv("WA_ENC_OVERLAP")) {
        const double per_layer = tm / (double)(p.k + 1);
        double fill = kEncOverlapFill;
        if (const char* e = getenv("WA_ENC_FILL")) fill = atof(e);
        m->overlap_k = std::max(0, std::min(L, (int)(fill * td / per_layer) - 1));
      }
    }
    if (const char* e = getenv("WA_ENC_OVERLAP")) m->overlap_k = std::max(0, std::min(L, atoi(e)));
    if (i + 1 < NU) {
      u.k = m->overlap_k;
      WA_HIP(hipStreamWaitEvent(es, u.ready, 0));
      WA_HIP(hipEventRecord(u.mstart, es));
      WA_TRY(encoder_front(m, mel_dev + ut[i + 1].first * mel_stride, B, es));
      WA_TRY(encoder_layers(m, B, 0, u.k, es));
      WA_HIP(hipEventRecord(u.mend, es));
    }
    WA_TRY(run_decode(m, B, pair, lang_token, max_tokens, eot_stop, u.ready, u.gprompt, u.gdone, u.gsteps));
    int32_t* hb = host + (size_t)u.first * per;
    WA_TRY(collect_batch(m, B, pair, u.gdone, st, hb, hb + (size_t)B * kMaxTokens, hb + (size_t)B * kMaxTokens + B,
                         per));
    if (i + 1 < NU) {
      WA_HIP(hipStreamWaitEvent(st, u.mend, 0));
      WA_HIP(hipEventRecord(u.pstart, st));
      WA_TRY(unit_encoder(ut[i + 1], u.k));
    }
  }
  WA_HIP(hipStreamSynchronize(st));
  hg.done = true;
  for (int i = 0; i < NB; ++i) {
    const int32_t* hb = host + (size_t)i * per;
    copy_tokens(hb, hb + (size_t)B * kMaxTokens, B, max_tokens, tokens_out + (size_t)i * B * max_tokens,
                n_tokens_out + (size_t)i * B);
    flags[i] = hb[(size_t)B * kMaxTokens + B];
  }
  for (int i = 0; i < NU; ++i) {
    Unit& u = ut[i];
    const int UG = unit_groups(B, u.n == 2);
    float t = 0.0f, tp = 0.0f, td = 0.0f;
    if (i == 0) {
      WA_HIP(hipEventElapsedTime(&t, e_enc0, u.ready));
    } else {
      WA_HIP(hipEventElapsedTime(&t, ut[i - 1].pstart, u.ready));
      float tm = 0.0f;
      WA_HIP(hipEventElapsedTime(&tm, ut[i - 1].mstart, ut[i - 1].mend));
      t_masked += tm;
      k_sum += ut[i - 1].k;
    }
    t_exposed += t;
    for (int g = 0; g < UG; ++g) {
      float a = 0.0f, d = 0.0f;
      WA_HIP(hipEventElapsedTime(&a, u.ready, u.gprompt[g]));
      WA_HIP(hipEventElapsedTime(&d, u.ready, u.gdone[g]));
      tp = std::max(tp, a);
      td = std::max(td, d);
    }
    t_prompt += tp;
    t_decode += td - tp;
    steps_all += u.n == 2 ? u.gsteps[0] + u.gsteps[1] : *std::max_element(u.gsteps, u.gsteps + UG);
  }
  m->timings[0] = (float)(t_exposed / NB);
  m->timings[1] = 0.0f;
  m->timings[2] = (float)(t_prompt / NB);
  m->timings[3] = (float)(t_decode / NB);
  m->timings[4] = (float)steps_all / NB;
  m->pipe[0] = (float)NB;
  m->pipe[1] = NU > 1 ? (float)(k_sum / (NU - 1)) : 0.0f;
  m->pipe[2] = NU > 1 ? (float)(t_masked / (NU - 1)) : 0.0f;
  m->pipe[3] = (float)m->enc_cus;
  m->pipe_pairs = pairing ? NB / 2 : 0;
  return WQ4_OK;
}

}

extern "C" {

wq4_status wa_transcribe(wa_model* m, const float* mel_dev, int n_clips, int lang_token, int max_tokens,
                         int eot_stop, int32_t* tokens_out, int32_t* n_tokens_out, void* stream) {
  if (!m || !mel_dev || !tokens_out || !n_tokens_out) return fail(WQ4_EINVAL, "null argument");
  if (n_clips < 1 || n_clips > m->bmax) return fail(WQ4_EINVAL, "n_clips out of range");
  if (max_tokens < 1 || max_tokens > kMaxTokens) return fail(WQ4_EINVAL, "max_tokens must be in [1, 224]");
  WA_HIP(hipSetDevice(m->device));
  for (;;) {
    bool overflow = false;
    WA_TRY(transcribe_once(m, mel_dev, n_clips, lang_token, max_tokens, eot_stop, tokens_out, n_tokens_out, stream,
                           &overflow));
    if (!overflow) return WQ4_OK;
    if (m->range_tier == 3)
      return fail(WQ4_ERANGE,
                  "activation overflow: an MFMA operand left the f16-pair range (|x| >= 4094 after every range tier: "
                  "LayerNorm path, per-call FFN and attention-projection operand scales) and the logits are not finite");
    if (m->range_tier == 1) WA_TRY(ensure_ffn_ws(m));
    ++m->range_tier;
  }
}

wq4_status wa_transcribe_batches(wa_model* m, const float* mel_dev, int n_batches, int n_clips, int lang_token,
                                 int max_tokens, int eot_stop, int32_t* tokens_out, int32_t* n_tokens_out,
                                 void* stream) {
  if (!m || !mel_dev || !tokens_out || !n_tokens_out) return fail(WQ4_EINVAL, "null argument");
  if (n_batches < 1) return fail(WQ4_EINVAL, "n_batches must be >= 1");
  if (n_clips < 1 || n_clips > m->bmax) return fail(WQ4_EINVAL, "n_clips out of range");
  if (max_tokens < 1 || max_tokens > kMaxTokens) return fail(WQ4_EINVAL, "max_tokens must be in [1, 224]");
  WA_HIP(hipSetDevice(m->device));
  std::vector<int> flags(n_batches, 0);
  WA_TRY(transcribe_pipelined(m, mel_dev, n_batches, n_clips, lang_token, max_tokens, eot_stop, tokens_out,
                              n_tokens_out, stream, flags.data()));
  const size_t mel_stride = (size_t)n_clips * m->cfg.n_mels * 2 * m->cfg.n_audio_ctx;
  const int tier0 = m->range_tier;
  for (int i = 0; i < n_batches; ++i) {
    if (!flags[i] && m->range_tier == tier0) continue;
    WA_TRY(wa_transcribe(m, mel_dev + i * mel_stride, n_clips, lang_token, max_tokens, eot_stop,
                         tokens_out + (size_t)i * n_clips * max_tokens, n_tokens_out + (size_t)i * n_clips, stream));
  }
  return WQ4_OK;
}

wq4_status wa_last_pipeline_stats(const wa_model* m, float* out) {
  if (!m || !out) return fail(WQ4_EINVAL, "null argument");
  std::memcpy(out, m->pipe, sizeof(m->pipe));
  return WQ4_OK;
}

int wa_last_pipeline_pairs(const wa_model* m) { return m ? m->pipe_pairs : 0; }

wq4_status wa_transcribe_trace(wa_model* m, const float* mel_dev, int n_clips, int lang_token, int max_tokens,
                               int eot_stop, int32_t* tokens_out, int32_t* n_tokens_out, const int32_t* trace_ids_dev,
                               int trace_k, float* trace_out_dev, void* stream) {
  if (!m || !trace_ids_dev || !trace_out_dev || trace_k < 1) return fail(WQ4_EINVAL, "bad trace arguments");
  m->trace_ids = trace_ids_dev;
  m->trace_out = trace_out_dev;
  m->trace_s1 = max_tokens + 1;
  m->trace_k = trace_k;
  const wq4_status s = wa_transcribe(m, mel_dev, n_clips, lang_token, max_tokens, eot_stop, tokens_out,
                                     n_tokens_out, stream);
  m->trace_ids = nullptr;
  m->trace_out = nullptr;
  m->trace_s1 = m->trace_k = 0;
  for (DecGroup& g : m->groups) {
    for (hipGraphExec_t* x : {&g.graph, &g.graph_alt}) {
      if (*x) (void)hipGraphExecDestroy(*x);
      *x = nullptr;
    }
    g.graph_key = g.graph_alt_key = -1;
  }
  return s;
}

}
```

### whisper-burn_amd/csrc/whisper/wa_xattn.hip

```cpp
#include <hip/hip_runtime.h>

#include <algorithm>
#include <cmath>
#include <cstdlib>
#include <type_traits>

#include "../wq4_device.hpp"
#include "../wq4_lnmath.hpp"
#include "wa_kernels.hpp"

namespace wa {
namespace {

using wq4::atile_store4;
using wq4::attn_store4;
using wq4::kbp_of;
using wq4::split_f16;
using wq4::half2v;
typedef _Float16 half4 __attribute__((ext_vector_type(4)));
typedef float floatx4 __attribute__((ext_vector_type(4)));
typedef float floatx2 __attribute__((ext_vector_type(2)));

constexpr int kWtQ4 = 0, kWtF16 = 1;
constexpr int kTc = 16;
constexpr int kMaxD = 1280;
constexpr float kXqScale = 0.125f * 1.4426950408889634f;
constexpr float kWkScale = 4096.0f, kXqInv = 1.0f / (16.0f * 4096.0f);
constexpr float kQtScale = 32.0f, kEncScale = 32.0f, kSInv = 1.0f / 1024.0f;
constexpr float kPScale = 16384.0f, kZInv = 1.0f / (16384.0f * 32.0f);
constexpr float kZnScale = 32.0f, kWvScale = 4096.0f, kOutInv = 1.0f / (32.0f * 4096.0f);
#ifndef WA_XATTN_SPLITS
#define WA_XATTN_SPLITS 8
#endif
constexpr int kXattnSplits = WA_XATTN_SPLITS;
#ifndef WA_XATTN_DIAG
#define WA_XATTN_DIAG 0
#endif
#ifndef WA_XATTN_CACHE_FRAMES
#define WA_XATTN_CACHE_FRAMES 1500
#endif
#ifndef WA_XATTN_STREAM_AUX
#define WA_XATTN_STREAM_AUX 2
#endif
constexpr int kMaxFrames = 1500;
#ifndef WA_XATTN_STAMP
#define WA_XATTN_STAMP 0
#endif
#if WA_XATTN_STAMP
constexpr int kXsPhases = 8, kXsChunks = 16;
__device__ unsigned long long g_xstamp[2][kXsChunks][kXsPhases];
#endif
#ifndef WA_XATTN_ODIAG
#define WA_XATTN_ODIAG 0
#endif

typedef _Float16 half8 __attribute__((ext_vector_type(8)));
typedef float floatx16 __attribute__((ext_vector_type(16)));
typedef __fp16 fp16x4_t __attribute__((__vector_size__(4 * sizeof(__fp16))));

__device__ __forceinline__ floatx4 mfma16x32(half8 a, half8 b, floatx4 c) {
  return __builtin_amdgcn_mfma_f32_16x16x32_f16(a, b, c, 0, 0, 0);
}
__device__ __forceinline__ floatx16 mfma32x16(half8 a, half8 b, floatx16 c) {
  return __builtin_amdgcn_mfma_f32_32x32x16_f16(a, b, c, 0, 0, 0);
}
__device__ __forceinline__ half4 lds_tr4(const _Float16* p) {
  return __builtin_bit_cast(half4, __builtin_amdgcn_ds_read_tr16_b64_v4f16(
                                       (__attribute__((address_space(3))) fp16x4_t*)(p)));
}

template <int WK>
__device__ __forceinline__ void load_w32(const uint8_t* __restrict__ w, int K, int o, int kb, float* out) {
  if (WK == kWtQ4) {
    const uint16_t* blk = reinterpret_cast<const uint16_t*>(w + ((size_t)o * (K / 32) + kb) * 18);
    const float d = (float)__builtin_bit_cast(_Float16, blk[0]);
#pragma unroll
    for (int i = 0; i < 8; ++i) {
      const uint32_t two = blk[1 + i];
      out[2 * i] = (float)((int)(two & 15u) - 8) * d;
      out[2 * i + 1] = (float)((int)((two >> 8) & 15u) - 8) * d;
      out[16 + 2 * i] = (float)((int)((two >> 4) & 15u) - 8) * d;
      out[16 + 2 * i + 1] = (float)((int)((two >> 12) & 15u) - 8) * d;
    }
  } else {
    const _Float16* p = reinterpret_cast<const _Float16*>(w) + (size_t)o * K + kb * 32;
#pragma unroll
    for (int i = 0; i < 32; ++i) out[i] = (float)p[i];
  }
}

template <int NS, int WK>
__global__ __launch_bounds__(128) void xattn_q_mfma_kernel(const float* __restrict__ q, int R, int D,
                                                           const uint8_t* __restrict__ wk, int HP,
                                                           _Float16* __restrict__ qt) {
  constexpr int LD = 72;
  __shared__ __attribute__((aligned(16))) _Float16 wth[64 * LD];
  __shared__ __attribute__((aligned(16))) _Float16 wtl[64 * LD];
  const int h = blockIdx.x, c0 = blockIdx.y * 64, r0 = blockIdx.z * 32, tid = threadIdx.x;
  const int w = tid >> 6, l = tid & 63, l32 = l & 31, kh = l >> 5;
  const int row = r0 + l32;
  floatx4 xa[4][2];
#pragma unroll
  for (int ks = 0; ks < 4; ++ks)
#pragma unroll
    for (int u = 0; u < 2; ++u)
      xa[ks][u] = row < R ? *reinterpret_cast<const floatx4*>(q + (size_t)row * D + h * 64 + ks * 16 + 8 * kh + 4 * u)
                          : floatx4{0.0f, 0.0f, 0.0f, 0.0f};
  {
    const int d = tid >> 1, b = tid & 1;
    float v[32];
    load_w32<WK>(wk, D, h * 64 + d, (c0 >> 5) + b, v);
#pragma unroll
    for (int i = 0; i < 32; ++i) {
      _Float16 hi, lo;
      split_f16(v[i] * kWkScale, hi, lo);
      wth[(b * 32 + i) * LD + d] = hi;
      wtl[(b * 32 + i) * LD + d] = lo;
    }
  }
  half8 ah[4], al[4];
#pragma unroll
  for (int ks = 0; ks < 4; ++ks)
#pragma unroll
    for (int j = 0; j < 8; ++j) {
      _Float16 x, y;
      wq4::split_act(xa[ks][j >> 2][j & 3], x, y);
      ah[ks][j] = x;
      al[ks][j] = y;
    }
  __syncthreads();
  floatx16 acc = {};
  const int c = 32 * w + l32;
#pragma unroll
  for (int ks = 0; ks < 4; ++ks) {
    const half8 bh = *reinterpret_cast<const half8*>(&wth[c * LD + ks * 16 + 8 * kh]);
    const half8 bl = *reinterpret_cast<const half8*>(&wtl[c * LD + ks * 16 + 8 * kh]);
    acc = mfma32x16(ah[ks], bh, acc);
    acc = mfma32x16(al[ks], bh, acc);
    acc = mfma32x16(ah[ks], bl, acc);
  }
#pragma unroll
  for (int i = 0; i < 16; ++i) {
    const int r = r0 + (i & 3) + 8 * (i >> 2) + 4 * kh;
    if (r < R) {
      _Float16 x, y;
      split_f16(acc[i] * kXqInv * kXqScale * kQtScale, x, y);
      qt[(((size_t)r * NS + 0) * HP + h) * D + c0 + c] = x;
      if (NS == 2) qt[(((size_t)r * NS + 1) * HP + h) * D + c0 + c] = y;
    }
  }
}

constexpr float kLazyMax = 1024.0f;
__device__ __forceinline__ void softmax_entry(float sv, bool valid, float& M, float& L, float& alpha, float& p) {
  sv = valid ? sv : -INFINITY;
  const float cm = wq4::max16(sv);
  float mn = fmaxf(M, cm);
  if (M != -INFINITY && mn - M <= kLazyMax) mn = M;
  alpha = 1.0f;
  p = 0.0f;
  if (mn != -INFINITY) {
    alpha = __builtin_amdgcn_exp2f((M - mn) * kSInv);
    p = valid ? __builtin_amdgcn_exp2f((sv - mn) * kSInv) : 0.0f;
  }
  const float ps = wq4::sum16(p);
  L = L * alpha + ps;
  M = mn;
}

template <int D, int HT, int NS, int NW, int PF>
__global__ __launch_bounds__(64 * NW) void xattn_main_kernel(const _Float16* __restrict__ qt,
                                                             const _Float16* __restrict__ enc, int Tq, int T,
                                                             int H, int S, int CH, float* __restrict__ zpart,
                                                             float* __restrict__ mlpart, int R) {
  constexpr int kThreads = 64 * NW;
  constexpr int CW = D / NW;
  constexpr int KS = CW / 32;
  constexpr int HP = HT * 16;
  constexpr int ROW = NS * D;
  constexpr int RS = ROW + 32;
  constexpr int NV = kTc * ROW / 8;
  constexpr int NLD = (NV + kThreads - 1) / kThreads;
  constexpr int HR = HT == 2 ? 1 : HT;
  static_assert(CW * NW == D && CW % 32 == 0 && HT <= 2 && (PF == 1 || PF == 2), "bad column split");
  __shared__ __attribute__((aligned(16))) _Float16 se[kTc * RS];
  __shared__ __attribute__((aligned(16))) float red[NW][HT][16][20];
  __shared__ __attribute__((aligned(16))) _Float16 sp[NS][32][kTc + 8];
  __shared__ float salpha[32];
  __shared__ int srescale[2];
  __shared__ __attribute__((aligned(16))) _Float16 sq1[HT == 2 ? NS : 1][5][HT == 2 ? D + 16 : 8];

  const int s = blockIdx.x, r = blockIdx.y;
  const int tid = threadIdx.x, w = tid >> 6, l = tid & 63;
  const int l16 = l & 15, lq = l >> 4, l32 = l & 31, lh = l >> 5;
  const _Float16* E = enc + (size_t)(r / Tq) * T * ROW;
  const int c0 = w * CW;
  const int ts = s * CH * kTc;
  const int te = min(T, ts + CH * kTc);
  const int nch = WA_XATTN_DIAG == 10 ? 0 : te > ts ? (te - ts + kTc - 1) / kTc : 0;
#if WA_XATTN_STAMP
  const int stamp_w = (s == 0 && r == 0 && l == 0) ? (w == 0 ? 0 : w == NW - 1 ? 1 : -1) : -1;
  auto stamp = [&](int chi, int ph) {
    asm volatile("s_waitcnt vmcnt(0) lgkmcnt(0)" ::: "memory");
    const unsigned long long t = __builtin_readcyclecounter();
    if (stamp_w >= 0 && chi < kXsChunks) g_xstamp[stamp_w][chi][ph] = t;
  };
#else
  auto stamp = [](int, int) {};
#endif

  half8 qb[HR][KS][NS];
#pragma unroll
  for (int ht = 0; ht < HR; ++ht)
#pragma unroll
    for (int ks = 0; ks < KS; ++ks)
#pragma unroll
      for (int p = 0; p < NS; ++p)
        qb[ht][ks][p] = *reinterpret_cast<const half8*>(
            qt + (((size_t)r * NS + p) * HP + ht * 16 + l16) * D + c0 + ks * 32 + 8 * lq);
  if (HT == 2) {
    for (int i = tid; i < NS * 5 * (D / 8); i += kThreads) {
      const int p = i / (5 * (D / 8)), rem = i - p * 5 * (D / 8), hr = rem / (D / 8), c8 = rem - hr * (D / 8);
      *reinterpret_cast<half8*>(&sq1[p][hr][8 * c8]) =
          hr < 4 ? *reinterpret_cast<const half8*>(qt + (((size_t)r * NS + p) * HP + 16 + hr) * D + 8 * c8) : half8{};
    }
  }
  for (int i = tid; i < NS * 32 * (kTc + 8); i += kThreads) (&sp[0][0][0])[i] = (_Float16)(WA_XATTN_DIAG == 9 ? 1.0f : 0.0f);
  if (tid < 32) salpha[tid] = 1.0f;
  if (tid < 2) srescale[tid] = 0;

  floatx16 zacc[KS];
#pragma unroll
  for (int ct = 0; ct < KS; ++ct)
#pragma unroll
    for (int j = 0; j < 16; ++j) zacc[ct][j] = 0.0f;
  constexpr int SMX = (HT * 256 + kThreads - 1) / kThreads;
  float M[SMX], L[SMX];
#pragma unroll
  for (int e = 0; e < SMX; ++e) {
    M[e] = -INFINITY;
    L[e] = 0.0f;
  }

  typedef uint32_t u32x4v __attribute__((ext_vector_type(4)));
  constexpr int PPR = CW / 8;
  static_assert(NLD * 64 == NS * kTc * PPR, "the slice is a whole number of loads per lane");
  const __amdgpu_buffer_rsrc_t rs = __builtin_amdgcn_make_buffer_rsrc(
      const_cast<_Float16*>(E + (size_t)ts * ROW), 0, nch > 0 ? (te - ts) * ROW * 2 : 0, 0x00020000);
  auto item = [&](int i, int& row, int& col) {
    const int v = l + 64 * i;
    const int p = v / (kTc * PPR), rem = v - p * (kTc * PPR);
    row = rem / PPR;
    col = p * D + c0 + (rem - row * PPR) * 8;
  };
  auto fetch_aux = [&](u32x4v(&buf)[NLD], int chi, auto aux_c) {
#pragma unroll
    for (int i = 0; i < NLD; ++i) {
      int row, col;
      item(i, row, col);
      buf[i] = __builtin_amdgcn_raw_buffer_load_b128(rs, (uint32_t)(((chi * kTc + row) * ROW + col) * 2), 0,
                                                     decltype(aux_c)::value);
    }
  };
  auto fetch = [&](u32x4v (&buf)[NLD], int chi) {
    if (WA_XATTN_CACHE_FRAMES >= kMaxFrames || ts + chi * kTc < WA_XATTN_CACHE_FRAMES)
      fetch_aux(buf, chi, std::integral_constant<int, 0>{});
    else
      fetch_aux(buf, chi, std::integral_constant<int, WA_XATTN_STREAM_AUX>{});
  };

  const int g = l >> 4, gi = l & 15;
  const int trow = 8 * (g >> 1) + (gi >> 2), tcol = 16 * (g & 1) + 4 * (gi & 3);
  auto sw = [](int t) { return (t & 8) ? 3 : 0; };
  const int lq_sw = lq ^ sw(l16);
  auto write_se = [&](const u32x4v (&buf)[NLD]) {
#pragma unroll
    for (int i = 0; i < NLD; ++i) {
      int row, col;
      item(i, row, col);
      *reinterpret_cast<u32x4v*>(&se[row * RS + (((col >> 3) ^ sw(row)) << 3)]) = buf[i];
    }
  };

  const int q1row = l16 < 4 ? l16 : 4;
  auto b1frag = [&](int ks, int p) {
    return *reinterpret_cast<const half8*>(&sq1[p][q1row][c0 + ks * 32 + 8 * lq]);
  };
  auto scores = [&](auto&& afrag) {
    floatx4 sacc[HT];
#pragma unroll
    for (int ht = 0; ht < HT; ++ht) sacc[ht] = floatx4{0.0f, 0.0f, 0.0f, 0.0f};
#pragma unroll
    for (int ks = 0; ks < (WA_XATTN_DIAG == 3 ? 0 : KS); ++ks) {
      half8 a[NS], b1[NS];
#pragma unroll
      for (int p = 0; p < NS; ++p) {
        a[p] = afrag(ks, p);
        if (HT > HR) b1[p] = b1frag(ks, p);
      }
#pragma unroll
      for (int ht = 0; ht < HT; ++ht) {
        half8 b[NS];
#pragma unroll
        for (int p = 0; p < NS; ++p) b[p] = ht < HR ? qb[ht < HR ? ht : 0][ks][p] : b1[p];
        sacc[ht] = mfma16x32(a[0], b[0], sacc[ht]);
        if constexpr (NS == 2) {
          sacc[ht] = mfma16x32(a[1], b[0], sacc[ht]);
          sacc[ht] = mfma16x32(a[0], b[1], sacc[ht]);
        }
      }
    }
#pragma unroll
    for (int ht = 0; ht < HT; ++ht) *reinterpret_cast<floatx4*>(&red[w][ht][l16][4 * lq]) = sacc[ht];
  };
  auto softmax_phase = [&](int chi, int t0) {
#pragma unroll
    for (int e = 0; e < SMX; ++e) {
      const int idx = tid + e * kThreads;
      if (idx < HT * 256 && WA_XATTN_DIAG != 4 && WA_XATTN_DIAG != 9) {
        const int ht = idx >> 8, hh = (idx >> 4) & 15, t = idx & 15;
        const int h = ht * 16 + hh;
        float sv = 0.0f;
#pragma unroll
        for (int ww = 0; ww < NW; ++ww) sv += red[ww][ht][hh][t];
        const bool valid = h < H && t0 + t < te;
        float alpha, p;
        softmax_entry(sv, valid, M[e], L[e], alpha, p);
        _Float16 phi, plo;
        split_f16(p * kPScale, phi, plo);
        if (WA_XATTN_DIAG == 8) phi = plo = (_Float16)0.0f;
        sp[0][h][t] = phi;
        if (NS == 2) sp[1][h][t] = plo;
        if (t == 0) salpha[h] = alpha;
        if (alpha != 1.0f && WA_XATTN_DIAG != 5) srescale[chi & 1] = 1;
      }
    }
  };
  auto z_phase = [&](int chi) {
    const bool rescale = srescale[chi & 1] != 0;
    if (tid == 0) srescale[(chi + 1) & 1] = 0;
    half8 pa[NS];
#pragma unroll
    for (int p = 0; p < NS; ++p) pa[p] = *reinterpret_cast<const half8*>(&sp[p][l32][8 * lh]);
    if (rescale) {
#pragma unroll
      for (int j = 0; j < 16; ++j) {
        const float al = salpha[(j & 3) + 8 * (j >> 2) + 4 * lh];
#pragma unroll
        for (int ct = 0; ct < KS; ++ct) zacc[ct][j] *= al;
      }
    }
    stamp(chi, 6);
    const int tc0 = ((((tcol >> 3) ^ sw(trow)) << 3) | (tcol & 7));
    const int tc1 = ((((tcol >> 3) ^ sw(trow + 4)) << 3) | (tcol & 7));
#pragma unroll
    for (int ct = 0; ct < (WA_XATTN_DIAG == 2 ? 0 : KS); ++ct) {
      half8 eb[NS];
#pragma unroll
      for (int p = 0; p < NS; ++p) {
        const half4 x0 = lds_tr4(&se[trow * RS + p * D + c0 + ct * 32 + tc0]);
        const half4 x1 = lds_tr4(&se[(trow + 4) * RS + p * D + c0 + ct * 32 + tc1]);
        eb[p] = half8{x0[0], x0[1], x0[2], x0[3], x1[0], x1[1], x1[2], x1[3]};
      }
      zacc[ct] = mfma32x16(pa[0], eb[0], zacc[ct]);
      if (NS == 2) {
        zacc[ct] = mfma32x16(pa[1], eb[0], zacc[ct]);
        zacc[ct] = mfma32x16(pa[0], eb[1], zacc[ct]);
      }
    }
  };
  auto step = [&](u32x4v (&buf)[NLD], int chi) {
    const int t0 = ts + chi * kTc;
    stamp(chi, 0);
    write_se(buf);
    stamp(chi, 1);
    if (chi + PF < nch && WA_XATTN_DIAG != 1) fetch(buf, chi + PF);
    scores([&](int ks, int p) {
      return *reinterpret_cast<const half8*>(&se[l16 * RS + p * D + c0 + ks * 32 + 8 * lq_sw]);
    });
    stamp(chi, 2);
    if (WA_XATTN_DIAG != 6) __syncthreads();
    stamp(chi, 3);
    softmax_phase(chi, t0);
    stamp(chi, 4);
    if (WA_XATTN_DIAG != 7) __syncthreads();
    stamp(chi, 5);
    z_phase(chi);
    stamp(chi, 7);
  };
  u32x4v pre0[NLD];
  u32x4v pre1[PF == 2 ? NLD : 1];
  if (nch > 0) fetch(pre0, 0);
  __syncthreads();
  if constexpr (PF == 2) {
    if (nch > 1) fetch(pre1, 1);
    for (int chi = 0; chi < nch; chi += 2) {
      step(pre0, chi);
      if (chi + 1 < nch) step(pre1, chi + 1);
    }
  } else {
    for (int chi = 0; chi < nch; ++chi) step(pre0, chi);
  }

  const size_t base = (size_t)r * S + s;
#pragma unroll
  for (int e = 0; e < SMX; ++e) {
    const int idx = tid + e * kThreads;
    if (idx < HT * 256 && (idx & 15) == 0) {
      const int h = (idx >> 8) * 16 + ((idx >> 4) & 15);
      if (h < H) {
        mlpart[(base * H + h) * 2] = M[e] * kSInv;
        mlpart[(base * H + h) * 2 + 1] = L[e];
      }
    }
  }
#pragma unroll
  for (int j = 0; j < 16; ++j) {
    const int h = (j & 3) + 8 * (j >> 2) + 4 * lh;
    if (h < H) {
#pragma unroll
      for (int ct = 0; ct < KS; ++ct) zpart[(base * H + h) * D + c0 + ct * 32 + l32] = zacc[ct][j] * kZInv;
    }
  }
}

constexpr int kWvPackU32 = 64 + 8;
__global__ __launch_bounds__(256) void wv_pack_kernel(const uint8_t* __restrict__ wv, int H, int D,
                                                      uint32_t* __restrict__ out) {
  const int64_t i = (int64_t)blockIdx.x * 256 + threadIdx.x;
  const int nkb = D / 32;
  if (i >= (int64_t)H * nkb * 4 * 64) return;
  const int l = (int)(i & 63), mt = (int)((i >> 6) & 3);
  const int64_t hk = i >> 8;
  const int kb = (int)(hk % nkb), h = (int)(hk / nkb);
  const int n = l & 15, lq = l >> 4;
  const uint8_t* blk = wv + ((size_t)h * 64 + mt * 16 + n) * ((size_t)nkb * 18) + (size_t)kb * 18;
  uint32_t wd = 0;
#pragma unroll
  for (int j = 0; j < 8; ++j) {
    const int e = 8 * lq + j;
    const uint32_t q = e < 16 ? (blk[2 + e] & 15u) : (blk[2 + e - 16] >> 4);
    wd |= q << (4 * j);
  }
  uint32_t* o = out + (((size_t)h * nkb + kb) * 4 + mt) * kWvPackU32;
  o[l] = wd;
  if (lq == 0) reinterpret_cast<uint16_t*>(o + 64)[n] = (uint16_t)(blk[0] | (blk[1] << 8));
}

template <int NS, int WK, int RPW, int SM, int MTG>
__global__ __launch_bounds__(512) void xattn_out_kernel(const float* __restrict__ zpart,
                                                        const float* __restrict__ mlpart, int R, int H, int D, int S,
                                                        const uint8_t* __restrict__ wv,
                                                        const uint32_t* __restrict__ wvp,
                                                        const float* __restrict__ bv, _Float16* __restrict__ tiled,
                                                        float* __restrict__ out32) {
  constexpr int ZLD = kMaxD + 8;
  __shared__ __attribute__((aligned(16))) uint8_t zbuf[WK == kWtQ4 ? 2 * RPW * ZLD * 2 : kMaxD * RPW * 4];
  float* zs = reinterpret_cast<float*>(zbuf);
  _Float16* zh = reinterpret_cast<_Float16*>(zbuf);
  _Float16* zl = zh + RPW * ZLD;
  __shared__ __attribute__((aligned(16))) _Float16 zzero[8];
  __shared__ float red[16][64][RPW + 1];
  static_assert(MTG == 1 || WK == kWtQ4, "output groups need the Q4 MFMA projection");
  constexpr int NMT = 4 / MTG;
  const int h = blockIdx.x, rbase = blockIdx.y * RPW, rstep = 1, mt0 = blockIdx.z * NMT;
  const int tid = threadIdx.x;
  const int nkb = D / 32;
  const float bias1 = tid < 16 * NMT * RPW ? bv[h * 64 + 16 * mt0 + (tid & (16 * NMT - 1))] : 0.0f;
  constexpr int KPW = kMaxD / 32 / 8;
  uint32_t wq[WK == kWtQ4 ? KPW : 1][WK == kWtQ4 ? NMT : 1], wd[WK == kWtQ4 ? KPW : 1][WK == kWtQ4 ? NMT : 1];
  if constexpr (WK == kWtQ4) {
    const int l = tid & 63, w = tid >> 6;
#pragma unroll
    for (int u = 0; u < KPW; ++u) {
      const int kb = w + 8 * u < nkb ? w + 8 * u : 0;
#pragma unroll
      for (int mt = 0; mt < NMT; ++mt) {
        const uint32_t* o = wvp + (((size_t)h * nkb + kb) * 4 + mt0 + mt) * kWvPackU32;
        wq[u][mt] = WA_XATTN_ODIAG == 1 ? 0u : o[l];
        wd[u][mt] = WA_XATTN_ODIAG == 1 ? 0u : reinterpret_cast<const uint16_t*>(o + 64)[l & 15];
      }
    }
  }
  __shared__ float swt[RPW][SM + 1];
  {
    const int nq = D / 4;
    constexpr int NIT = (RPW * (kMaxD / 4) + 511) / 512;
    floatx4 zv[NIT][SM];
#pragma unroll
    for (int u = 0; u < NIT; ++u) {
      const int it = tid + 512 * u;
      const int j = it / nq, q = it - j * nq;
      const bool ok = it < RPW * nq && rbase + rstep * j < R;
      const size_t rb = (size_t)(ok ? rbase + rstep * j : 0) * S;
      const floatx4* zp = reinterpret_cast<const floatx4*>(zpart + (rb * H + h) * D) + (ok ? q : 0);
#pragma unroll
      for (int s = 0; s < SM; ++s)
        if (s < S) zv[u][s] = WA_XATTN_ODIAG == 2 ? floatx4{0.0f, 0.0f, 0.0f, 0.0f} : zp[(size_t)s * H * (D / 4)];
    }
    if (tid < RPW) {
      const int j = tid;
      const size_t rb = (size_t)(rbase + rstep * j < R ? rbase + rstep * j : 0) * S;
      const floatx2* mp = reinterpret_cast<const floatx2*>(mlpart) + rb * H + h;
      floatx2 ml[SM];
#pragma unroll
      for (int s = 0; s < SM; ++s)
        if (s < S) ml[s] = WA_XATTN_ODIAG == 2 ? floatx2{0.0f, 1.0f} : mp[(size_t)s * H];
      float mx = -INFINITY;
#pragma unroll
      for (int s = 0; s < SM; ++s)
        if (s < S) mx = fmaxf(mx, ml[s][0]);
      float lsum = 0.0f;
#pragma unroll
      for (int s = 0; s < SM; ++s)
        if (s < S) {
          const float w = ml[s][0] == -INFINITY ? 0.0f : __builtin_amdgcn_exp2f(ml[s][0] - mx);
          lsum = fmaf(w, ml[s][1], lsum);
          swt[j][s] = w;
        }
      swt[j][SM] = lsum;
    }
    __syncthreads();
#pragma unroll
    for (int u = 0; u < NIT; ++u) {
      const int it = tid + 512 * u;
      if (it >= RPW * nq) break;
      const int j = it / nq, q = it - j * nq;
      const bool rok = rbase + rstep * j < R;
      floatx4 acc = {0.0f, 0.0f, 0.0f, 0.0f};
#pragma unroll
      for (int s = 0; s < SM; ++s)
        if (s < S) {
          const float w = swt[j][s];
#pragma unroll
          for (int e = 0; e < 4; ++e) acc[e] = fmaf(w, zv[u][s][e], acc[e]);
        }
      const float lsum = swt[j][SM];
      if constexpr (WK == kWtQ4) {
        half4 hi, lo;
#pragma unroll
        for (int e = 0; e < 4; ++e) {
          _Float16 x, y;
          split_f16(rok ? acc[e] / lsum * kZnScale : 0.0f, x, y);
          hi[e] = x;
          lo[e] = y;
        }
        *reinterpret_cast<half4*>(&zh[j * ZLD + 4 * q]) = hi;
        *reinterpret_cast<half4*>(&zl[j * ZLD + 4 * q]) = lo;
      } else {
#pragma unroll
        for (int e = 0; e < 4; ++e) zs[(4 * q + e) * RPW + j] = rok ? acc[e] / lsum : 0.0f;
      }
    }
  }
  if (tid < 8) zzero[tid] = (_Float16)0.0f;
  __syncthreads();
  constexpr int NPART = WK == kWtQ4 ? 8 : 16;
  if constexpr (WK == kWtQ4) {
    const int w = tid >> 6, l = tid & 63, n = l & 15, lq = l >> 4;
    floatx4 acc[4];
#pragma unroll
    for (int mt = 0; mt < NMT; ++mt) acc[mt] = floatx4{0.0f, 0.0f, 0.0f, 0.0f};
#pragma unroll
    for (int u = 0; u < KPW; ++u) {
      const int kb = w + 8 * u;
      if (kb >= (WA_XATTN_ODIAG == 3 ? 0 : nkb)) break;
      const _Float16* zhp = n < RPW ? &zh[n * ZLD + kb * 32 + 8 * lq] : zzero;
      const _Float16* zlp = n < RPW ? &zl[n * ZLD + kb * 32 + 8 * lq] : zzero;
      const half8 bh = *reinterpret_cast<const half8*>(zhp);
      const half8 bl = *reinterpret_cast<const half8*>(zlp);
#pragma unroll
      for (int mt = 0; mt < NMT; ++mt) {
        const _Float16 d = __builtin_bit_cast(_Float16, (uint16_t)wd[u][mt]) * (_Float16)kWvScale;
        const half2v off = {(_Float16)1032.0f, (_Float16)1032.0f};
        const half2v dv = {d, d};
        half8 ah, al;
#pragma unroll
        for (int i = 0; i < 4; ++i) {
          const uint32_t x = wq[u][mt] >> (8 * i);
          const uint32_t pr = (x & 0xFu) | ((x << 12) & 0xF0000u) | 0x64006400u;
          const half2v qv = __builtin_bit_cast(half2v, pr) - off;
          const half2v hv = qv * dv;
          const half2v lv = __builtin_elementwise_fma(qv, dv, -hv);
          ah[2 * i] = hv[0];
          ah[2 * i + 1] = hv[1];
          al[2 * i] = lv[0];
          al[2 * i + 1] = lv[1];
        }
        acc[mt] = mfma16x32(ah, bh, acc[mt]);
        acc[mt] = mfma16x32(ah, bl, acc[mt]);
        acc[mt] = mfma16x32(al, bh, acc[mt]);
      }
    }
    if (n < RPW) {
#pragma unroll
      for (int mt = 0; mt < NMT; ++mt)
#pragma unroll
        for (int i = 0; i < 4; ++i) red[w][16 * mt + 4 * lq + i][n] = acc[mt][i];
    }
  } else {
    const int dp = tid & 31, bg = tid >> 5;
    float acc0[RPW], acc1[RPW];
#pragma unroll
    for (int j = 0; j < RPW; ++j) {
      acc0[j] = 0.0f;
      acc1[j] = 0.0f;
    }
#pragma unroll 1
    for (int kb = bg; kb < nkb; kb += 16) {
      float w0[32], w1[32];
      load_w32<WK>(wv, D, h * 64 + dp, kb, w0);
      load_w32<WK>(wv, D, h * 64 + dp + 32, kb, w1);
#pragma unroll
      for (int i = 0; i < 32; ++i) {
        const float* z = &zs[(kb * 32 + i) * RPW];
#pragma unroll
        for (int j = 0; j < RPW; ++j) {
          acc0[j] = fmaf(w0[i], z[j], acc0[j]);
          acc1[j] = fmaf(w1[i], z[j], acc1[j]);
        }
      }
    }
#pragma unroll
    for (int j = 0; j < RPW; ++j) {
      red[bg][dp][j] = acc0[j];
      red[bg][dp + 32][j] = acc1[j];
    }
  }
  __syncthreads();
  if (tid < 16 * NMT * RPW) {
    const int j = tid / (16 * NMT), d = tid & (16 * NMT - 1), r = rbase + rstep * j;
    float sacc = bias1;
#pragma unroll
    for (int g = 0; g < NPART; ++g) sacc += red[g][d][j] * (WK == kWtQ4 ? kOutInv : 1.0f);
    const float v1 = __shfl_down(sacc, 1, 64), v2 = __shfl_down(sacc, 2, 64), v3 = __shfl_down(sacc, 3, 64);
    if (r < R && (d & 3) == 0) attn_store4<NS>(tiled, out32, D, r, h * 64 + 16 * mt0 + d, kbp_of(D), sacc, v1, v2, v3);
  }
}

template <int NS>
__global__ __launch_bounds__(256) void enc_planes_kernel(const float* __restrict__ x, int64_t n, int D,
                                                         _Float16* __restrict__ out) {
  const int64_t i = (int64_t)blockIdx.x * 256 + threadIdx.x;
  if (i >= n) return;
  const int64_t row = i / D;
  const int c = (int)(i - row * D);
  _Float16 hi, lo;
  split_f16(x[i] * kEncScale, hi, lo);
  out[(row * NS) * D + c] = hi;
  if (NS == 2) out[(row * NS + 1) * D + c] = lo;
}

template <int NS>
__global__ __launch_bounds__(256) void untile_kernel(const _Float16* __restrict__ t, int R, int K,
                                                     float* __restrict__ out) {
  const int i = blockIdx.x * 256 + threadIdx.x;
  if (i >= R * K) return;
  const int r = i / K, k = i - r * K;
  float v = (float)t[wq4::atile_index(r, k, kbp_of(K), NS, 0)];
  if (NS == 2) v += (float)t[wq4::atile_index(r, k, kbp_of(K), NS, 1)];
  out[i] = v * wq4::kActScaleInv;
}

constexpr int kSmallMaxCH = 12;
constexpr int kSmallRowsMax = 8;

template <int D, int HT, int NS, int NW>
__global__ __launch_bounds__(64 * NW) void xattn_scores_kernel(const _Float16* __restrict__ qt,
                                                               const _Float16* __restrict__ enc, int Tq, int T,
                                                               int NG, float* __restrict__ sbuf) {
  constexpr int CW = D / NW, KS = CW / 32, HP = HT * 16, ROW = NS * D;
  __shared__ __attribute__((aligned(16))) float red[NW][HT][16][20];
  const int g = blockIdx.x, r = blockIdx.y;
  const int tid = threadIdx.x, w = tid >> 6, l = tid & 63, l16 = l & 15, lq = l >> 4;
  const int c0 = w * CW, f = g * kTc + l16;
  const _Float16* E = enc + (size_t)(r / Tq) * T * ROW;
  half8 a[KS][NS];
  const int fc = f < T ? f : T - 1;
#pragma unroll
  for (int ks = 0; ks < KS; ++ks)
#pragma unroll
    for (int p = 0; p < NS; ++p)
      a[ks][p] = *reinterpret_cast<const half8*>(E + (size_t)fc * ROW + p * D + c0 + ks * 32 + 8 * lq);
  if (f >= T) {
#pragma unroll
    for (int ks = 0; ks < KS; ++ks)
#pragma unroll
      for (int p = 0; p < NS; ++p) a[ks][p] = half8{};
  }
  half8 qb[KS][HT][NS];
#pragma unroll
  for (int ks = 0; ks < KS; ++ks)
#pragma unroll
    for (int ht = 0; ht < HT; ++ht) {
      const int hr = (HT == 2 && ht == 1) ? 16 + (l16 & 3) : ht * 16 + l16;
#pragma unroll
      for (int p = 0; p < NS; ++p)
        qb[ks][ht][p] = *reinterpret_cast<const half8*>(qt + (((size_t)r * NS + p) * HP + hr) * D + c0 + ks * 32 + 8 * lq);
    }
  __builtin_amdgcn_sched_barrier(0);
  floatx4 sacc[HT];
#pragma unroll
  for (int ht = 0; ht < HT; ++ht) sacc[ht] = floatx4{0.0f, 0.0f, 0.0f, 0.0f};
#pragma unroll
  for (int ks = 0; ks < KS; ++ks)
#pragma unroll
    for (int ht = 0; ht < HT; ++ht) {
      const bool ok = !(HT == 2 && ht == 1) || l16 < 4;
      half8 b[NS];
#pragma unroll
      for (int p = 0; p < NS; ++p) b[p] = ok ? qb[ks][ht][p] : half8{};
      sacc[ht] = mfma16x32(a[ks][0], b[0], sacc[ht]);
      if constexpr (NS == 2) {
        sacc[ht] = mfma16x32(a[ks][1], b[0], sacc[ht]);
        sacc[ht] = mfma16x32(a[ks][0], b[1], sacc[ht]);
      }
    }
#pragma unroll
  for (int ht = 0; ht < HT; ++ht) *reinterpret_cast<floatx4*>(&red[w][ht][l16][4 * lq]) = sacc[ht];
  __syncthreads();
  for (int idx = tid; idx < HT * 256; idx += 64 * NW) {
    const int ht = idx >> 8, hh = (idx >> 4) & 15, t = idx & 15;
    float sv = 0.0f;
#pragma unroll
    for (int ww = 0; ww < NW; ++ww) sv += red[ww][ht][hh][t];
    sbuf[(((size_t)r * NG + g) * HP + ht * 16 + hh) * 16 + t] = sv;
  }
}

template <int D, int HT, int NS>
__global__ __launch_bounds__(256) void xattn_z_kernel(const _Float16* __restrict__ enc,
                                                      const float* __restrict__ sbuf, int Tq, int T, int H, int S,
                                                      int CH, int NG, float* __restrict__ zpart,
                                                      float* __restrict__ mlpart) {
  constexpr int ROW = NS * D, ZR = 32, HP = HT * 16;
  constexpr int SMX = 512 / 256;
  __shared__ __attribute__((aligned(16))) _Float16 sp[kSmallMaxCH][NS][32][kTc];
  __shared__ float sal[kSmallMaxCH][32];
  __shared__ int sfl[kSmallMaxCH];
  __shared__ __attribute__((aligned(16))) _Float16 stg[4][NS][16 * ZR];
  const int s = blockIdx.x, r = blockIdx.z, tid = threadIdx.x, w = tid >> 6, l = tid & 63;
  const int l32 = l & 31, lh = l >> 5;
  const int cb = blockIdx.y * 128 + w * 32;
  const int ts = s * CH * kTc, te = min(T, ts + CH * kTc);
  const int nch = te > ts ? (te - ts + kTc - 1) / kTc : 0;
  const size_t g0 = (size_t)r * NG + s * CH;
  typedef uint32_t u32x4v __attribute__((ext_vector_type(4)));
  const _Float16* E = enc + (size_t)(r / Tq) * T * ROW;
  const __amdgpu_buffer_rsrc_t rs = __builtin_amdgcn_make_buffer_rsrc(
      const_cast<_Float16*>(E + (size_t)ts * ROW), 0, nch > 0 ? (te - ts) * ROW * 2 : 0, 0x00020000);
  u32x4v ev[kSmallMaxCH][NS];
#pragma unroll
  for (int c = 0; c < kSmallMaxCH; ++c)
#pragma unroll
    for (int p = 0; p < NS; ++p)
      ev[c][p] = __builtin_amdgcn_raw_buffer_load_b128(
          rs, (uint32_t)((((c * kTc + (l >> 2)) * ROW) + p * D + cb + 8 * (l & 3)) * 2), 0, 0);
  float sv_all[kSmallMaxCH][SMX];
#pragma unroll
  for (int c = 0; c < kSmallMaxCH; ++c)
#pragma unroll
    for (int e = 0; e < SMX; ++e) {
      const int idx = tid + e * 256, h = idx >> 4, t = idx & 15;
      const int cc = c < nch ? c : 0, hc = h < HP ? h : 0;
      sv_all[c][e] = sbuf[((g0 + cc) * HP + hc) * 16 + t];
    }
  if (tid < kSmallMaxCH) sfl[tid] = 0;
  __syncthreads();
  float M[SMX], L[SMX];
#pragma unroll
  for (int e = 0; e < SMX; ++e) {
    M[e] = -INFINITY;
    L[e] = 0.0f;
  }
#pragma unroll
  for (int chi = 0; chi < kSmallMaxCH; ++chi) {
    if (chi >= nch) continue;
    const int t0 = ts + chi * kTc;
#pragma unroll
    for (int e = 0; e < SMX; ++e) {
      const int idx = tid + e * 256, h = idx >> 4, t = idx & 15;
      _Float16 phi = (_Float16)0.0f, plo = (_Float16)0.0f;
      float alpha = 1.0f;
      if (h < HP) {
        float p;
        softmax_entry(sv_all[chi][e], h < H && t0 + t < te, M[e], L[e], alpha, p);
        split_f16(p * kPScale, phi, plo);
      }
      sp[chi][0][h][t] = phi;
      if (NS == 2) sp[chi][1][h][t] = plo;
      if (t == 0) sal[chi][h] = alpha;
      if (alpha != 1.0f) sfl[chi] = 1;
    }
  }
  if (blockIdx.y == 0) {
    const size_t base = (size_t)r * S + s;
#pragma unroll
    for (int e = 0; e < SMX; ++e) {
      const int idx = tid + e * 256, h = idx >> 4;
      if ((idx & 15) == 0 && h < H && h < HP) {
        mlpart[(base * H + h) * 2] = M[e] * kSInv;
        mlpart[(base * H + h) * 2 + 1] = L[e];
      }
    }
  }
  __syncthreads();
  const int g = l >> 4, gi = l & 15;
  const int trow = 8 * (g >> 1) + (gi >> 2), tcol = 16 * (g & 1) + 4 * (gi & 3);
  floatx16 zacc;
#pragma unroll
  for (int j = 0; j < 16; ++j) zacc[j] = 0.0f;
#pragma unroll
  for (int chi = 0; chi < kSmallMaxCH; ++chi) {
    if (chi >= nch) continue;
#pragma unroll
    for (int p = 0; p < NS; ++p)
      *reinterpret_cast<u32x4v*>(&stg[w][p][(l >> 2) * ZR + 8 * (l & 3)]) = ev[chi][p];
    half8 pa[NS];
#pragma unroll
    for (int p = 0; p < NS; ++p) pa[p] = *reinterpret_cast<const half8*>(&sp[chi][p][l32][8 * lh]);
    if (sfl[chi]) {
#pragma unroll
      for (int j = 0; j < 16; ++j) zacc[j] *= sal[chi][(j & 3) + 8 * (j >> 2) + 4 * lh];
    }
    half8 eb[NS];
#pragma unroll
    for (int p = 0; p < NS; ++p) {
      const half4 x0 = lds_tr4(&stg[w][p][trow * ZR + tcol]);
      const half4 x1 = lds_tr4(&stg[w][p][(trow + 4) * ZR + tcol]);
      eb[p] = half8{x0[0], x0[1], x0[2], x0[3], x1[0], x1[1], x1[2], x1[3]};
    }
    zacc = mfma32x16(pa[0], eb[0], zacc);
    if (NS == 2) {
      zacc = mfma32x16(pa[1], eb[0], zacc);
      zacc = mfma32x16(pa[0], eb[1], zacc);
    }
  }
  const size_t base = (size_t)r * S + s;
#pragma unroll
  for (int j = 0; j < 16; ++j) {
    const int h = (j & 3) + 8 * (j >> 2) + 4 * lh;
    if (h < H) zpart[(base * H + h) * D + cb + l32] = zacc[j] * kZInv;
  }
}

template <int D, int HT, int NS>
void launch_small(int R, int Tq, int T, int H, const XattnPlan& p, const _Float16* qt, const _Float16* enc,
                  float* z, float* ml, float* scratch, hipStream_t st) {
  constexpr int NW = (D / 8) % 32 == 0 ? 8 : 4;
  const int NG = p.splits * p.ch;
  float* sb = scratch;
  hipLaunchKernelGGL((xattn_scores_kernel<D, HT, NS, NW>), dim3(NG, R), dim3(64 * NW), 0, st, qt, enc, Tq, T, NG, sb);
  hipLaunchKernelGGL((xattn_z_kernel<D, HT, NS>), dim3(p.splits, D / 128, R), dim3(256), 0, st, enc, sb, Tq, T, H,
                     p.splits, p.ch, NG, z, ml);
}

int xattn_small_rows() {
  int v = 4;
  if (const char* e = getenv("WA_XATTN_SMALL_ROWS")) v = atoi(e);
  return std::max(0, std::min(kSmallRowsMax, v));
}

template <int D, int HT, int NS>
void launch_main(dim3 g, const _Float16* qt, const _Float16* enc, int Tq, int T, int H, int S, int CH, float* z,
                 float* ml, int R, hipStream_t st) {
  constexpr int NW = (D / 8) % 32 == 0 ? 8 : 4;
  hipLaunchKernelGGL((xattn_main_kernel<D, HT, NS, NW, 1>), g, dim3(64 * NW), 0, st, qt, enc, Tq, T, H, S, CH, z, ml,
                     R);
}

#ifndef WA_XATTN_OUT_ROWS
#define WA_XATTN_OUT_ROWS 4
#endif
int out_rows(int R) {
  (void)R;
  return WA_XATTN_OUT_ROWS;
}
template <int NS, int WK, int RPW>
void launch_out_rpw(int R, int H, const float* z, const float* ml, int D, int S, const uint8_t* wv,
                    const uint32_t* wvp, const float* bv, _Float16* tiled, float* out32, hipStream_t st,
                    bool split_outputs) {
  const dim3 go(H, (R + RPW - 1) / RPW);
  if constexpr (WK == kWtQ4) {
    if (split_outputs) {
      hipLaunchKernelGGL((xattn_out_kernel<NS, WK, RPW, kXattnSplits, 4>), dim3(go.x, go.y, 4), dim3(512), 0, st, z,
                         ml, R, H, D, S, wv, wvp, bv, tiled, out32);
      return;
    }
  }
  hipLaunchKernelGGL((xattn_out_kernel<NS, WK, RPW, kXattnSplits, 1>), go, dim3(512), 0, st, z, ml, R, H, D, S, wv,
                     wvp, bv, tiled, out32);
}
template <int NS, int WK>
void launch_out(int R, int H, const float* z, const float* ml, int D, int S, const uint8_t* wv, const uint32_t* wvp,
                const float* bv, _Float16* tiled, float* out32, hipStream_t st, bool split_outputs = false) {
  switch (out_rows(R)) {
    case 1: launch_out_rpw<NS, WK, 1>(R, H, z, ml, D, S, wv, wvp, bv, tiled, out32, st, split_outputs); break;
    case 2: launch_out_rpw<NS, WK, 2>(R, H, z, ml, D, S, wv, wvp, bv, tiled, out32, st, split_outputs); break;
    case 8: launch_out_rpw<NS, WK, 8>(R, H, z, ml, D, S, wv, wvp, bv, tiled, out32, st, split_outputs); break;
    default: launch_out_rpw<NS, WK, 4>(R, H, z, ml, D, S, wv, wvp, bv, tiled, out32, st, split_outputs); break;
  }
}

}

XattnPlan xattn_plan(int R, int T) {
  (void)R;
  const int nchunk = (T + kTc - 1) / kTc;
  const int S = std::max(1, std::min(kXattnSplits, nchunk));
  XattnPlan p;
  p.ch = (nchunk + S - 1) / S;
  p.splits = (nchunk + p.ch - 1) / p.ch;
  return p;
}

size_t xattn_part_floats(int R, int H, int D, int T) {
  const XattnPlan p = xattn_plan(R, T);
  size_t n = (size_t)R * p.splits * H * ((size_t)D + 2) + (size_t)R * H * D;
  if (R <= kSmallRowsMax) {
    const size_t ng = (size_t)p.splits * p.ch;
    n = (n + 3) / 4 * 4 + (size_t)R * ng * 32 * 16 + 4;
  }
  return n;
}

hipError_t launch_untile(const _Float16* tiled, int R, int K, int ns, float* out, hipStream_t st) {
  const dim3 g((R * K + 255) / 256);
  if (ns == 2)
    hipLaunchKernelGGL(untile_kernel<2>, g, dim3(256), 0, st, tiled, R, K, out);
  else
    hipLaunchKernelGGL(untile_kernel<1>, g, dim3(256), 0, st, tiled, R, K, out);
  return hipGetLastError();
}

hipError_t launch_enc_planes(const float* x, int64_t rows, int D, int ns, _Float16* out, hipStream_t st) {
  const int64_t n = rows * D;
  const dim3 g((unsigned)((n + 255) / 256));
  if (ns == 2)
    hipLaunchKernelGGL(enc_planes_kernel<2>, g, dim3(256), 0, st, x, n, D, out);
  else
    hipLaunchKernelGGL(enc_planes_kernel<1>, g, dim3(256), 0, st, x, n, D, out);
  return hipGetLastError();
}

size_t wv_pack_words(int H, int D) { return (size_t)H * (D / 32) * 4 * kWvPackU32; }

hipError_t launch_wv_pack(const uint8_t* wv, int H, int D, uint32_t* out, hipStream_t st) {
  if (D % 32 != 0 || D > kMaxD) return hipErrorInvalidValue;
  const int64_t n = (int64_t)H * (D / 32) * 4 * 64;
  hipLaunchKernelGGL(wv_pack_kernel, dim3((unsigned)((n + 255) / 256)), dim3(256), 0, st, wv, H, D, out);
  return hipGetLastError();
}

hipError_t launch_xattn(const float* q, const uint8_t* wk, const uint8_t* wv, const uint32_t* wvp, const float* bv,
                        int wtype, const _Float16* enc, int B, int Tq, int T, int H, int D, _Float16* qt, float* part,
                        _Float16* tiled, int ns, hipStream_t st, float* out32) {
  const int R = B * Tq;
  const int HT = (H + 15) / 16, HP = HT * 16;
  if (D != H * 64 || D % 128 != 0 || D > kMaxD || H > 20 || !q) return hipErrorInvalidValue;
  if (wtype == kWtQ4 && !wvp) return hipErrorInvalidValue;
  const XattnPlan p = xattn_plan(R, T);
  float* z = part;
  float* ml = part + (size_t)R * p.splits * H * D;
  const dim3 gq(H, D / 64, (R + 31) / 32);
#define WA_XQ(NS_, WK_) hipLaunchKernelGGL((xattn_q_mfma_kernel<NS_, WK_>), gq, dim3(128), 0, st, q, R, D, wk, HP, qt)
  if (wtype == kWtQ4) {
    if (ns == 2) WA_XQ(2, kWtQ4); else WA_XQ(1, kWtQ4);
  } else {
    if (ns == 2) WA_XQ(2, kWtF16); else WA_XQ(1, kWtF16);
  }
#undef WA_XQ
  const dim3 gm(p.splits, R);
  const bool small = R <= xattn_small_rows() && p.ch <= kSmallMaxCH;
  float* scratch = part + ((size_t)R * p.splits * H * ((size_t)D + 2) + (size_t)R * H * D + 3) / 4 * 4;
#define WA_XMAIN(DD, HH)                                                                   \
  if (D == DD && HT == HH) {                                                               \
    if (small) {                                                                           \
      if (ns == 2)                                                                         \
        launch_small<DD, HH, 2>(R, Tq, T, H, p, qt, enc, z, ml, scratch, st);              \
      else                                                                                 \
        launch_small<DD, HH, 1>(R, Tq, T, H, p, qt, enc, z, ml, scratch, st);              \
    } else if (ns == 2)                                                                    \
      launch_main<DD, HH, 2>(gm, qt, enc, Tq, T, H, p.splits, p.ch, z, ml, R, st);          \
    else                                                                                   \
      launch_main<DD, HH, 1>(gm, qt, enc, Tq, T, H, p.splits, p.ch, z, ml, R, st);          \
  } else
  WA_XMAIN(1280, 2)
  WA_XMAIN(1024, 1)
  WA_XMAIN(768, 1)
  WA_XMAIN(512, 1)
  WA_XMAIN(384, 1)
  return hipErrorInvalidValue;
#undef WA_XMAIN
  if (wtype == kWtQ4) {
    if (ns == 2)
      launch_out<2, kWtQ4>(R, H, z, ml, D, p.splits, wv, wvp, bv, tiled, out32, st, small);
    else
      launch_out<1, kWtQ4>(R, H, z, ml, D, p.splits, wv, wvp, bv, tiled, out32, st, small);
  } else {
    if (ns == 2)
      launch_out<2, kWtF16>(R, H, z, ml, D, p.splits, wv, wvp, bv, tiled, out32, st, small);
    else
      launch_out<1, kWtF16>(R, H, z, ml, D, p.splits, wv, wvp, bv, tiled, out32, st, small);
  }
  return hipGetLastError();
}

}
```

### whisper-burn_amd/whisper_amd/__init__.py

```python
from __future__ import annotations

import ctypes
import os
from typing import Optional

import numpy as np

import wq4

LIB_PATH = os.path.join(os.path.dirname(wq4.LIB_PATH), "libwhisper_amd.so")
HEADER_PATH = os.path.join(os.path.dirname(wq4.HEADER_PATH), "whisper_amd.h")
VARIANTS = {"large_v3": 0, "medium": 1, "tiny_test": 2}
CFG_KEYS = ["n_mels", "n_audio_ctx", "n_audio_state", "n_audio_head", "n_audio_layer", "n_text_ctx",
            "n_text_state", "n_text_head", "n_text_layer", "n_vocab", "n_lang"]
_lib: Optional[ctypes.CDLL] = None


def lib() -> ctypes.CDLL:
    global _lib
    if _lib is None:
        wq4.lib()
        if not os.path.exists(LIB_PATH):
            raise wq4.WQ4Error(6, f"{LIB_PATH} not built")
        L = ctypes.CDLL(LIB_PATH, mode=ctypes.RTLD_GLOBAL)
        vp, c_int, c_i64 = ctypes.c_void_p, ctypes.c_int, ctypes.c_int64
        i32p = ctypes.POINTER(ctypes.c_int32)
        f32p = ctypes.POINTER(ctypes.c_float)
        L.wa_last_error.restype = ctypes.c_char_p
        L.wa_model_create_synthetic.argtypes = [c_int, c_int, ctypes.c_uint64, c_int, c_int, ctypes.POINTER(vp)]
        L.wa_model_destroy.argtypes = [vp]
        L.wa_model_destroy.restype = None
        L.wa_model_config.argtypes = [vp, i32p]
        L.wa_model_device_bytes.argtypes = [vp]
        L.wa_model_device_bytes.restype = ctypes.c_size_t
        L.wa_transcribe.argtypes = [vp, vp, c_int, c_int, c_int, c_int, i32p, i32p, vp]
        L.wa_last_timings.argtypes = [vp, f32p]
        L.wa_transcribe_batches.argtypes = [vp, vp, c_int, c_int, c_int, c_int, c_int, i32p, i32p, vp]
        L.wa_last_pipeline_stats.argtypes = [vp, f32p]
        L.wa_last_pipeline_pairs.argtypes = [vp]
        L.wa_last_pipeline_pairs.restype = c_int
        L.wa_encode.argtypes = [vp, vp, c_int, vp, vp]
        L.wa_prompt_logits.argtypes = [vp, vp, c_int, c_int, vp, vp]
        L.wa_synth_uniform.argtypes = [ctypes.c_uint64, ctypes.c_char_p, c_i64, ctypes.c_float, ctypes.c_float, f32p]
        L.wa_profile_enable.argtypes = [vp, c_int]
        L.wa_profile_read.argtypes = [vp, ctypes.POINTER(ctypes.c_double), c_int]
        L.wa_probe_kernels.argtypes = [vp, c_int, c_int, ctypes.POINTER(ctypes.c_double), c_int]
        L.wa_decode_group_rows.argtypes = [c_int]
        L.wa_decode_group_rows.restype = c_int
        L.wa_model_create_synthetic_ex.argtypes = [c_int, c_int, ctypes.c_uint64, c_int, c_int, c_int,
                                                   ctypes.POINTER(vp)]
        L.wa_model_weight_type.argtypes = [vp]
        L.wa_model_weight_type.restype = c_int
        L.wa_model_wide_range.argtypes = [vp]
        L.wa_model_wide_range.restype = c_int
        L.wa_model_create_from_gguf.argtypes = [c_int, ctypes.c_char_p, c_int, c_int, c_int, ctypes.POINTER(vp)]
        L.wa_gguf_open.argtypes = [ctypes.c_char_p, ctypes.POINTER(vp)]
        L.wa_gguf_close.argtypes = [vp]
        L.wa_gguf_close.restype = None
        L.wa_gguf_version.argtypes = [vp]
        L.wa_gguf_version.restype = c_int
        L.wa_gguf_tensor_count.argtypes = [vp]
        L.wa_gguf_tensor_count.restype = c_i64
        L.wa_gguf_tensor_info.argtypes = [vp, c_i64, ctypes.c_char_p, ctypes.c_size_t, ctypes.POINTER(c_int),
                                          ctypes.POINTER(ctypes.c_uint64), ctypes.POINTER(c_int),
                                          ctypes.POINTER(ctypes.c_uint64), ctypes.POINTER(ctypes.c_uint64)]
        L.wa_gguf_tensor_data.argtypes = [vp, ctypes.c_char_p, ctypes.POINTER(ctypes.c_uint8), ctypes.c_size_t]
        L.wa_log_mel.argtypes = [c_int, vp, c_int, c_i64, c_i64, c_int, vp, vp]
        L.wa_mel_filterbank.argtypes = [c_int, f32p, f32p]
        L.wa_xattn_check.argtypes = [c_int, vp, vp, vp, vp, c_int, vp, c_int, c_int, c_int, c_int, c_int, vp]
        L.wa_xattn_kv_check.argtypes = [c_int, vp, vp, vp, c_int, c_int, c_int, c_int, c_int, vp]
        L.wa_transcribe_trace.argtypes = [vp, vp, c_int, c_int, c_int, c_int, i32p, i32p, vp, c_int, vp, vp]
        L.wa_encoder_attention_check.argtypes = [c_int, vp, c_int, c_int, c_int, c_int, vp]
        L.wa_self_attention_check.argtypes = [c_int, vp, vp, vp, c_int, c_int, c_int, c_int, c_int, c_int, vp]
        L.wa_logits_argmax_check.argtypes = [c_int, vp, vp, c_int, c_int, c_int, c_int, c_int, vp, vp]
        for n in ("wa_xattn_check", "wa_xattn_kv_check", "wa_transcribe_trace", "wa_encoder_attention_check", "wa_self_attention_check",
                  "wa_logits_argmax_check", "wa_log_mel", "wa_mel_filterbank", "wa_model_create_synthetic", "wa_model_config", "wa_transcribe", "wa_transcribe_batches",
                  "wa_last_pipeline_stats", "wa_last_timings", "wa_encode",
                  "wa_prompt_logits", "wa_synth_uniform", "wa_profile_enable", "wa_profile_read", "wa_probe_kernels",
                  "wa_decode_group_rows",
                  "wa_model_create_from_gguf", "wa_model_create_synthetic_ex", "wa_gguf_open", "wa_gguf_tensor_info", "wa_gguf_tensor_data"):
            getattr(L, n).restype = c_int
        _lib = L
    return _lib


def check(st: int) -> None:
    if st != 0:
        raise wq4.WQ4Error(st, lib().wa_last_error().decode(errors="replace"))


def decode_group_rows(n_clips: int) -> int:
    return int(lib().wa_decode_group_rows(n_clips))


def synth_uniform(seed: int, name: str, n: int, lo: float, hi: float) -> np.ndarray:
    out = np.empty(n, np.float32)
    check(lib().wa_synth_uniform(seed, name.encode(), n, lo, hi, out.ctypes.data_as(ctypes.POINTER(ctypes.c_float))))
    return out


def _torch():
    import torch

    return torch


MEL_FRAMES = 3000
MEL_CHUNK = 480000


def mel_filterbank(n_mels: int = 128) -> tuple[np.ndarray, np.ndarray]:
    fb = np.empty((n_mels, 201), np.float32)
    win = np.empty(400, np.float32)
    f32p = ctypes.POINTER(ctypes.c_float)
    check(lib().wa_mel_filterbank(n_mels, fb.ctypes.data_as(f32p), win.ctypes.data_as(f32p)))
    return fb, win


def log_mel(audio, n_mels: int = 128, n_samples: Optional[int] = None, out=None):
    torch = _torch()
    assert audio.dtype == torch.float32 and audio.is_cuda and audio.dim() == 2
    if audio.stride(1) != 1:
        audio = audio.contiguous()
    B, L = audio.shape
    n = L if n_samples is None else int(n_samples)
    if out is None:
        out = torch.empty((B, n_mels, MEL_FRAMES), device=audio.device, dtype=torch.float32)
    dev = audio.device.index if audio.device.index is not None else torch.cuda.current_device()
    check(lib().wa_log_mel(dev, ctypes.c_void_p(audio.data_ptr()), B, n, audio.stride(0), n_mels,
                           ctypes.c_void_p(out.data_ptr()),
                           ctypes.c_void_p(torch.cuda.current_stream(audio.device).cuda_stream)))
    return out


def xattn_check(q, wk_raw, wv_raw, bv, enc, Tq: int, H: int, weight_type: int = 0,
                precision: int = wq4.PREC_F16X2):
    torch = _torch()
    B, T, D = enc.shape
    out = torch.empty((B * Tq, D), device=enc.device, dtype=torch.float32)
    dev = enc.device.index if enc.device.index is not None else 0
    ptr = lambda t: ctypes.c_void_p(t.contiguous().data_ptr())
    check(lib().wa_xattn_check(dev, ptr(q), ptr(wk_raw), ptr(wv_raw), ptr(bv), weight_type, ptr(enc), B, Tq, T, H,
                               precision, ptr(out)))
    return out


def xattn_kv_check(q, k, v, Tq: int, precision: int = wq4.PREC_F16X2):
    torch = _torch()
    B, H, T, _ = k.shape
    out = torch.empty((B * Tq, 64 * H), device=k.device, dtype=torch.float32)
    dev = k.device.index if k.device.index is not None else 0
    ptr = lambda t: ctypes.c_void_p(t.contiguous().data_ptr())
    check(lib().wa_xattn_kv_check(dev, ptr(q), ptr(k), ptr(v), B, Tq, T, H, precision, ptr(out)))
    return out


def _dev(t) -> int:
    return t.device.index if t.device.index is not None else 0


def _ptr(t):
    return ctypes.c_void_p(t.data_ptr())


def encoder_attention_check(qkv, T: int, H: int, precision: int = wq4.PREC_F16X2):
    torch = _torch()
    qkv = qkv.contiguous()
    B = qkv.shape[0] // T
    out = torch.empty((B * T, 64 * H), device=qkv.device, dtype=torch.float32)
    check(lib().wa_encoder_attention_check(_dev(qkv), _ptr(qkv), B, T, H, precision, _ptr(out)))
    return out


def self_attention_check(qkv, cache_k, cache_v, Tq: int, H: int, kv_len: int, precision: int = wq4.PREC_F16X2):
    torch = _torch()
    B, _, ctx, _ = cache_k.shape
    out = torch.empty((B * Tq, 64 * H), device=qkv.device, dtype=torch.float32)
    check(lib().wa_self_attention_check(_dev(qkv), _ptr(qkv.contiguous()), _ptr(cache_k), _ptr(cache_v), B, Tq, H,
                                        ctx, kv_len, precision, _ptr(out)))
    return out


def logits_argmax_check(hid, emb, step: int, precision: int = wq4.PREC_F16X2, want_logits: bool = True):
    torch = _torch()
    B, D = hid.shape
    V = emb.shape[0]
    tok = torch.empty(B, device=hid.device, dtype=torch.int32)
    lg = torch.empty((B, V), device=hid.device, dtype=torch.float32) if want_logits else None
    check(lib().wa_logits_argmax_check(_dev(hid), _ptr(hid.contiguous()), _ptr(emb.contiguous()), B, D, V, step,
                                       precision, _ptr(tok), _ptr(lg) if lg is not None else None))
    return tok, lg


class GgufReader:

    def __init__(self, path: str):
        h = ctypes.c_void_p(None)
        check(lib().wa_gguf_open(path.encode(), ctypes.byref(h)))
        self._h = h

    @property
    def version(self) -> int:
        return lib().wa_gguf_version(self._h)

    def tensors(self) -> list[dict]:
        out = []
        for i in range(lib().wa_gguf_tensor_count(self._h)):
            name = ctypes.create_string_buffer(512)
            nd, ty = ctypes.c_int(), ctypes.c_int()
            dims = (ctypes.c_uint64 * 8)()
            off, nb = ctypes.c_uint64(), ctypes.c_uint64()
            check(lib().wa_gguf_tensor_info(self._h, i, name, 512, ctypes.byref(nd), dims, ctypes.byref(ty),
                                            ctypes.byref(off), ctypes.byref(nb)))
            out.append({"name": name.value.decode(), "dims": list(dims[: nd.value]), "type": ty.value,
                        "offset": off.value, "nbytes": nb.value})
        return out

    def tensor_data(self, name: str) -> np.ndarray:
        info = next(t for t in self.tensors() if t["name"] == name)
        buf = np.empty(info["nbytes"], np.uint8)
        check(lib().wa_gguf_tensor_data(self._h, name.encode(), buf.ctypes.data_as(ctypes.POINTER(ctypes.c_uint8)),
                                         buf.size))
        return buf

    def close(self):
        if self._h and self._h.value:
            lib().wa_gguf_close(self._h)
            self._h = ctypes.c_void_p(None)

    def __del__(self):
        try:
            self.close()
        except Exception:
            pass


class WhisperModel:

    WEIGHTS = {"q4_0": 0, "f16": 1}

    def __init__(self, variant: str = "large_v3", seed: int = 1234, max_batch: int = 1, device: int = 0,
                 precision: int = wq4.PREC_F16X2, gguf_path: Optional[str] = None, weights: str = "q4_0"):
        h = ctypes.c_void_p(None)
        if gguf_path is None:
            check(lib().wa_model_create_synthetic_ex(device, VARIANTS[variant], seed, max_batch, precision,
                                                     self.WEIGHTS[weights], ctypes.byref(h)))
        else:
            check(lib().wa_model_create_from_gguf(device, gguf_path.encode(), VARIANTS[variant], max_batch,
                                                  precision, ctypes.byref(h)))
        self._h = h
        self.device = device
        self.variant = variant
        self.max_batch = max_batch
        cfg = (ctypes.c_int32 * len(CFG_KEYS))()
        check(lib().wa_model_config(h, cfg))
        self.config = dict(zip(CFG_KEYS, list(cfg)))
        self.weights = {0: "q4_0", 1: "f16"}[lib().wa_model_weight_type(h)]

    @classmethod
    def from_gguf(cls, path: str, variant: str = "large_v3", max_batch: int = 1, device: int = 0,
                  precision: int = wq4.PREC_F16X2) -> "WhisperModel":
        return cls(variant, 0, max_batch, device, precision, gguf_path=path)

    @property
    def wide_range(self) -> bool:
        return lib().wa_model_wide_range(self._h) >= 1

    @property
    def range_tier(self) -> int:
        return lib().wa_model_wide_range(self._h)

    def device_bytes(self) -> int:
        return int(lib().wa_model_device_bytes(self._h))

    def _stream(self):
        return ctypes.c_void_p(_torch().cuda.current_stream(self.device).cuda_stream)

    def transcribe(self, mel, lang_token: Optional[int] = 50259, max_tokens: int = 224, eot_stop: bool = True):
        torch = _torch()
        mel = mel.contiguous()
        assert mel.dtype == torch.float32 and mel.is_cuda
        B = mel.shape[0]
        toks = np.zeros((B, max_tokens), np.int32)
        nt = np.zeros(B, np.int32)
        i32p = ctypes.POINTER(ctypes.c_int32)
        check(lib().wa_transcribe(self._h, ctypes.c_void_p(mel.data_ptr()), B,
                                  -1 if lang_token is None else int(lang_token), max_tokens, 1 if eot_stop else 0,
                                  toks.ctypes.data_as(i32p), nt.ctypes.data_as(i32p), self._stream()))
        return [toks[b, : nt[b]].tolist() for b in range(B)]

    def transcribe_batches(self, mels, lang_token: Optional[int] = 50259, max_tokens: int = 224,
                           eot_stop: bool = True):
        torch = _torch()
        mels = mels.contiguous()
        assert mels.dtype == torch.float32 and mels.is_cuda and mels.dim() == 4
        NB, B = mels.shape[0], mels.shape[1]
        toks = np.zeros((NB, B, max_tokens), np.int32)
        nt = np.zeros((NB, B), np.int32)
        i32p = ctypes.POINTER(ctypes.c_int32)
        check(lib().wa_transcribe_batches(self._h, ctypes.c_void_p(mels.data_ptr()), NB, B,
                                          -1 if lang_token is None else int(lang_token), max_tokens,
                                          1 if eot_stop else 0, toks.ctypes.data_as(i32p), nt.ctypes.data_as(i32p),
                                          self._stream()))
        return [[toks[i, b, : nt[i, b]].tolist() for b in range(B)] for i in range(NB)]

    def pipeline_stats(self) -> dict:
        t = (ctypes.c_float * 4)()
        check(lib().wa_last_pipeline_stats(self._h, t))
        return {"batches": int(t[0]), "overlap_layers": t[1], "masked_ms": t[2], "masked_cus": int(t[3])}

    def pipeline_pairs(self) -> int:
        return int(lib().wa_last_pipeline_pairs(self._h))

    def transcribe_trace(self, mel, trace_ids: np.ndarray, lang_token: Optional[int] = 50259,
                         max_tokens: int = 224, eot_stop: bool = False):
        torch = _torch()
        mel = mel.contiguous()
        B = mel.shape[0]
        K = trace_ids.shape[-1]
        assert trace_ids.shape == (B, max_tokens + 1, K)
        ids = torch.from_numpy(np.ascontiguousarray(trace_ids, np.int32)).to(mel.device)
        out = torch.full((B, max_tokens + 1, K), float("nan"), device=mel.device, dtype=torch.float32)
        toks = np.zeros((B, max_tokens), np.int32)
        nt = np.zeros(B, np.int32)
        i32p = ctypes.POINTER(ctypes.c_int32)
        check(lib().wa_transcribe_trace(self._h, _ptr(mel), B, -1 if lang_token is None else int(lang_token),
                                        max_tokens, 1 if eot_stop else 0, toks.ctypes.data_as(i32p),
                                        nt.ctypes.data_as(i32p), _ptr(ids), K, _ptr(out), self._stream()))
        return [toks[b, : nt[b]].tolist() for b in range(B)], out.cpu().numpy()

    def transcribe_audio(self, audio, lang_token: Optional[int] = 50259, max_tokens: int = 224,
                         eot_stop: bool = True, n_samples: Optional[int] = None):
        mel = log_mel(audio, self.config["n_mels"], n_samples)
        return self.transcribe(mel, lang_token, max_tokens, eot_stop)

    def last_timings(self) -> dict:
        t = (ctypes.c_float * 5)()
        check(lib().wa_last_timings(self._h, t))
        return {"encoder_ms": t[0], "cross_kv_ms": t[1], "prompt_ms": t[2], "decode_ms": t[3], "steps": int(t[4])}

    PROF_NAMES = ("q4_gemm", "encoder_attention", "conv", "layernorm")

    def profile_enable(self, on: bool = True) -> None:
        check(lib().wa_profile_enable(self._h, 1 if on else 0))

    def profile_read(self, reset: bool = True) -> dict:
        buf = (ctypes.c_double * 16)()
        check(lib().wa_profile_read(self._h, buf, 1 if reset else 0))
        return {n: {"launches": int(buf[4 * i]), "ms": buf[4 * i + 1], "gflop": buf[4 * i + 2], "gb": buf[4 * i + 3]}
                for i, n in enumerate(self.PROF_NAMES)}

    def probe_kernels(self, n_clips: int, iters: int = 20) -> dict:
        buf = (ctypes.c_double * 6)()
        check(lib().wa_probe_kernels(self._h, n_clips, iters, buf, len(buf)))
        return {"cross_attention": {"us": buf[0], "bytes": buf[1], "kv_cache": buf[5] != 0.0},
                "decode_fc1": {"us": buf[2], "bytes": buf[3], "flops": buf[4]}}

    def encode(self, mel):
        torch = _torch()
        B = mel.shape[0]
        out = torch.empty((B, self.config["n_audio_ctx"], self.config["n_audio_state"]), device=mel.device,
                          dtype=torch.float32)
        check(lib().wa_encode(self._h, ctypes.c_void_p(mel.contiguous().data_ptr()), B,
                              ctypes.c_void_p(out.data_ptr()), self._stream()))
        return out

    def prompt_logits(self, prompt):
        torch = _torch()
        B, T = prompt.shape
        out = torch.empty((B, self.config["n_vocab"]), device=prompt.device, dtype=torch.float32)
        check(lib().wa_prompt_logits(self._h, ctypes.c_void_p(prompt.contiguous().data_ptr()), B, T,
                                     ctypes.c_void_p(out.data_ptr()), self._stream()))
        return out

    def close(self):
        if self._h and self._h.value:
            lib().wa_model_destroy(self._h)
            self._h = ctypes.c_void_p(None)

    def __del__(self):
        try:
            self.close()
        except Exception:
            pass
```

Before: 1085.

## Partition cross-attention encoder chunks into cache-resident and streamed sets by live footprint

Adds a residency policy that estimates the live cross-attention encoder footprint across decode clips and, when it exceeds a cache budget, marks only a fraction of time chunks as cache-resident. The other chunks use streaming or nontemporal loads so they do not evict the resident set. The zpart partial buffers are now written and read with nontemporal hints to reduce cache pollution. The residency share is folded into the decode graph key, which can cause more graph rebuilds and relies on tuned budget constants.

```diff
diff --git a/include/whisper_amd.h b/include/whisper_amd.h
--- a/include/whisper_amd.h
+++ b/include/whisper_amd.h
@@ -81,6 +81,10 @@
 wq4_status wa_xattn_check(int device, const float* q_dev, const uint8_t* wk_dev, const uint8_t* wv_dev,
                           const float* bv_dev, int weight_type, const float* enc_dev, int n_clips, int Tq, int T,
                           int H, wq4_precision prec, float* out_dev);
+int wa_xattn_resident_share(int live_clips, int T, int planes, int D, double budget_mb);
+int wa_xattn_chunk_resident(int chunk, int share);
+wq4_status wa_xattn_plan(int T, int* splits, int* chunks_per_split);
+long long wa_decode_graph_key(const wa_model* m, int group);
 wq4_status wa_xattn_kv_check(int device, const float* q_dev, const float* k_dev, const float* v_dev, int n_clips,
                              int Tq, int T, int H, wq4_precision prec, float* out_dev);
 
diff --git a/whisper-burn_amd/csrc/whisper/wa_api.cpp b/whisper-burn_amd/csrc/whisper/wa_api.cpp
--- a/whisper-burn_amd/csrc/whisper/wa_api.cpp
+++ b/whisper-burn_amd/csrc/whisper/wa_api.cpp
@@ -178,6 +178,7 @@
   g.lane = 0;
   g.b0 = 0;
   g.nb = n_clips;
+  g.xres = xattn_residency(n_clips, m->cfg.n_audio_ctx, m->ns, m->cfg.n_audio_state);
   WA_TRY(decoder_forward(m, g, prompt_dev, plen, nullptr, 0, 0, st));
   WA_HIP(hipMemcpyAsync(logits_dev, g.logits, (size_t)n_clips * m->cfg.n_vocab * 4, hipMemcpyDeviceToDevice, st));
   return WQ4_OK;
@@ -210,11 +211,12 @@
   g.b0 = 0;
   g.nb = B;
   const bool kv = m->group_kv(g);
+  const XattnResidency res = xattn_residency(B, T, m->ns, D);
   auto xattn = [&]() -> hipError_t {
     if (kv)
       return launch_cross_attention_kv(g.qd, L.xk, L.xv, B, 1, T, H, g.xkv_part, g.xkv_ctr, g.atd_dec, m->ns, st);
     return launch_xattn(g.qd, L.ck_raw, L.cv_raw, L.cv_p, L.cv_b, m->wtype, enc, B, 1, T, H, D, g.xqt, g.xattn_part,
-                        g.atd_dec, m->ns, st);
+                        g.atd_dec, m->ns, res, st);
   };
   WA_HIP(xattn());
   WA_HIP(hipEventRecord(a, st));
diff --git a/whisper-burn_amd/csrc/whisper/wa_checks.cpp b/whisper-burn_amd/csrc/whisper/wa_checks.cpp
--- a/whisper-burn_amd/csrc/whisper/wa_checks.cpp
+++ b/whisper-burn_amd/csrc/whisper/wa_checks.cpp
@@ -47,10 +47,34 @@
     if (!wvp) return fail(WQ4_ENOMEM, "allocation failed");
     WA_HIP(launch_wv_pack(wv_dev, H, D, wvp, nullptr));
   }
+  const XattnResidency res = xattn_residency(n_clips, T, ns, D);
   return tiled_check(d, R, D, prec, out_dev, [&](_Float16* tiled) {
     return launch_xattn(q_dev, wk_dev, wv_dev, wvp, bv_dev, weight_type, enc, n_clips, Tq, T, H, D, qt, part, tiled,
-                        ns, nullptr);
-  });
+                        ns, res, nullptr);
+  });
+}
+
+int wa_xattn_resident_share(int live_clips, int T, int planes, int D, double budget_mb) {
+  if (live_clips < 1 || T < 1 || planes < 1 || planes > 2 || D < 1) return -1;
+  return xattn_residency(live_clips, T, planes, D, budget_mb).q;
+}
+
+int wa_xattn_chunk_resident(int chunk, int share) {
+  if (chunk < 0 || share < 0 || share > kXattnResDen) return -1;
+  return xattn_chunk_resident(chunk, share) ? 1 : 0;
+}
+
+wq4_status wa_xattn_plan(int T, int* splits, int* chunks_per_split) {
+  if (T < 1 || !splits || !chunks_per_split) return fail(WQ4_EINVAL, "bad arguments");
+  const XattnPlan p = xattn_plan(1, T);
+  *splits = p.splits;
+  *chunks_per_split = p.ch;
+  return WQ4_OK;
+}
+
+long long wa_decode_graph_key(const wa_model* m, int group) {
+  if (!m || group < 0 || group >= (int)m->groups.size()) return -1;
+  return m->groups[group].graph_key;
 }
 
 wq4_status wa_xattn_kv_check(int device, const float* q_dev, const float* k_dev, const float* v_dev, int n_clips,
diff --git a/whisper-burn_amd/csrc/whisper/wa_forward.cpp b/whisper-burn_amd/csrc/whisper/wa_forward.cpp
--- a/whisper-burn_amd/csrc/whisper/wa_forward.cpp
+++ b/whisper-burn_amd/csrc/whisper/wa_forward.cpp
@@ -333,7 +333,7 @@
                                        m->ns, st, a32));
     } else {
       WA_HIP(launch_xattn(g.qd, L.ck_raw, L.cv_raw, L.cv_p, L.cv_b, m->wtype, enc, B, Tq, T, H, D, g.xqt,
-                          g.xattn_part, g.atd_dec, m->ns, st, a32));
+                          g.xattn_part, g.atd_dec, m->ns, g.xres, st, a32));
     }
     WA_TRY(resid_gemm(L.cout, L.cout_b, g.atd_dec, a32, L.ln3_w));
     if (m->abi_ffn()) {
@@ -403,8 +403,8 @@
 
 wq4_status ensure_graph(wa_model* m, DecGroup& g, int eot_stop) {
   const int64_t key =
-      ((((((int64_t)g.lane * 512 + g.b0) * 512 + g.nb) * 2 + (eot_stop ? 1 : 0)) * 2 + (m->trace_out ? 1 : 0)) * 2 +
-       (m->group_kv(g) ? 1 : 0)) * 4 + m->range_tier;
+      (((((((int64_t)g.lane * 512 + g.b0) * 512 + g.nb) * 2 + (eot_stop ? 1 : 0)) * 2 + (m->trace_out ? 1 : 0)) * 2 +
+        (m->group_kv(g) ? 1 : 0)) * 4 + m->range_tier) * (kXattnResDen + 1) + g.xres.q;
   if (g.graph && g.graph_key == key) return WQ4_OK;
   std::swap(g.graph, g.graph_alt);
   std::swap(g.graph_key, g.graph_alt_key);
diff --git a/whisper-burn_amd/csrc/whisper/wa_kernels.hpp b/whisper-burn_amd/csrc/whisper/wa_kernels.hpp
--- a/whisper-burn_amd/csrc/whisper/wa_kernels.hpp
+++ b/whisper-burn_amd/csrc/whisper/wa_kernels.hpp
@@ -32,9 +32,15 @@
 size_t xattn_part_floats(int R, int H, int D, int T);
 size_t wv_pack_words(int H, int D);
 hipError_t launch_wv_pack(const uint8_t* wv, int H, int D, uint32_t* out, hipStream_t st);
+constexpr int kXattnResDen = 64;
+struct XattnResidency {
+  int q = kXattnResDen;
+};
+constexpr bool xattn_chunk_resident(int chunk, int q) { return ((chunk * q) & (kXattnResDen - 1)) + q >= kXattnResDen; }
+XattnResidency xattn_residency(int live_clips, int T, int ns, int D, double budget_mb = -1.0);
 hipError_t launch_xattn(const float* q, const uint8_t* wk, const uint8_t* wv, const uint32_t* wvp, const float* bv,
                         int wtype, const _Float16* enc, int B, int Tq, int T, int H, int D, _Float16* qt, float* part,
-                        _Float16* tiled, int ns, hipStream_t st, float* out32 = nullptr);
+                        _Float16* tiled, int ns, XattnResidency res, hipStream_t st, float* out32 = nullptr);
 hipError_t launch_untile(const _Float16* tiled, int R, int K, int ns, float* out, hipStream_t st);
 hipError_t launch_enc_planes(const float* x, int64_t rows, int D, int ns, _Float16* out, hipStream_t st);
 
diff --git a/whisper-burn_amd/csrc/whisper/wa_model.hpp b/whisper-burn_amd/csrc/whisper/wa_model.hpp
--- a/whisper-burn_amd/csrc/whisper/wa_model.hpp
+++ b/whisper-burn_amd/csrc/whisper/wa_model.hpp
@@ -89,6 +89,7 @@
   hipStream_t st = nullptr;
   int b0 = 0, nb = 0;
   int lane = 0;
+  XattnResidency xres;
   float *xd, *qkvd, *qd, *hid, *logits;
   _Float16 *atd_dec, *atf_dec;
   int *prompt_tok, *next_tok, *tokens, *ntok, *done;
diff --git a/whisper-burn_amd/csrc/whisper/wa_transcribe.cpp b/whisper-burn_amd/csrc/whisper/wa_transcribe.cpp
--- a/whisper-burn_amd/csrc/whisper/wa_transcribe.cpp
+++ b/whisper-burn_amd/csrc/whisper/wa_transcribe.cpp
@@ -38,8 +38,10 @@
 wq4_status run_decode(wa_model* m, int B, bool pair, int lang_token, int max_tokens, int eot_stop, hipEvent_t ready,
                       const hipEvent_t* gprompt, const hipEvent_t* gdone, int* gsteps) {
   const int G = unit_groups(B, pair);
+  const XattnResidency xres = xattn_residency(pair ? 2 * B : B, m->cfg.n_audio_ctx, m->ns, m->cfg.n_audio_state);
   for (int i = 0; i < G; ++i) {
     DecGroup& g = m->groups[i];
+    g.xres = xres;
     g.lane = pair ? i : 0;
     g.b0 = pair ? 0 : (int)((int64_t)B * i / G);
     g.nb = pair ? B : (int)((int64_t)B * (i + 1) / G) - g.b0;
diff --git a/whisper-burn_amd/csrc/whisper/wa_xattn.hip b/whisper-burn_amd/csrc/whisper/wa_xattn.hip
--- a/whisper-burn_amd/csrc/whisper/wa_xattn.hip
+++ b/whisper-burn_amd/csrc/whisper/wa_xattn.hip
@@ -36,13 +36,12 @@
 #ifndef WA_XATTN_DIAG
 #define WA_XATTN_DIAG 0
 #endif
-#ifndef WA_XATTN_CACHE_FRAMES
-#define WA_XATTN_CACHE_FRAMES 1500
-#endif
 #ifndef WA_XATTN_STREAM_AUX
 #define WA_XATTN_STREAM_AUX 2
 #endif
-constexpr int kMaxFrames = 1500;
+#ifndef WA_XATTN_ZPART_NT
+#define WA_XATTN_ZPART_NT 3
+#endif
 #ifndef WA_XATTN_STAMP
 #define WA_XATTN_STAMP 0
 #endif
@@ -168,11 +167,11 @@
   M = mn;
 }
 
-template <int D, int HT, int NS, int NW, int PF>
+template <int D, int HT, int NS, int NW, int PF, bool POL>
 __global__ __launch_bounds__(64 * NW) void xattn_main_kernel(const _Float16* __restrict__ qt,
                                                              const _Float16* __restrict__ enc, int Tq, int T,
                                                              int H, int S, int CH, float* __restrict__ zpart,
-                                                             float* __restrict__ mlpart, int R) {
+                                                             float* __restrict__ mlpart, int R, int resq) {
   constexpr int kThreads = 64 * NW;
   constexpr int CW = D / NW;
   constexpr int KS = CW / 32;
@@ -263,7 +262,7 @@
     }
   };
   auto fetch = [&](u32x4v (&buf)[NLD], int chi) {
-    if (WA_XATTN_CACHE_FRAMES >= kMaxFrames || ts + chi * kTc < WA_XATTN_CACHE_FRAMES)
+    if (!POL || xattn_chunk_resident(s * CH + chi, resq))
       fetch_aux(buf, chi, std::integral_constant<int, 0>{});
     else
       fetch_aux(buf, chi, std::integral_constant<int, WA_XATTN_STREAM_AUX>{});
@@ -419,7 +418,13 @@
     const int h = (j & 3) + 8 * (j >> 2) + 4 * lh;
     if (h < H) {
 #pragma unroll
-      for (int ct = 0; ct < KS; ++ct) zpart[(base * H + h) * D + c0 + ct * 32 + l32] = zacc[ct][j] * kZInv;
+      for (int ct = 0; ct < KS; ++ct) {
+        float* zp = &zpart[(base * H + h) * D + c0 + ct * 32 + l32];
+        if (WA_XATTN_ZPART_NT & 1)
+          __builtin_nontemporal_store(zacc[ct][j] * kZInv, zp);
+        else
+          *zp = zacc[ct][j] * kZInv;
+      }
     }
   }
 }
@@ -496,7 +501,10 @@
       const floatx4* zp = reinterpret_cast<const floatx4*>(zpart + (rb * H + h) * D) + (ok ? q : 0);
 #pragma unroll
       for (int s = 0; s < SM; ++s)
-        if (s < S) zv[u][s] = WA_XATTN_ODIAG == 2 ? floatx4{0.0f, 0.0f, 0.0f, 0.0f} : zp[(size_t)s * H * (D / 4)];
+        if (s < S)
+          zv[u][s] = WA_XATTN_ODIAG == 2         ? floatx4{0.0f, 0.0f, 0.0f, 0.0f}
+                     : (WA_XATTN_ZPART_NT & 2) ? __builtin_nontemporal_load(&zp[(size_t)s * H * (D / 4)])
+                                               : zp[(size_t)s * H * (D / 4)];
     }
     if (tid < RPW) {
       const int j = tid;
@@ -668,7 +676,7 @@
 template <int D, int HT, int NS, int NW>
 __global__ __launch_bounds__(64 * NW) void xattn_scores_kernel(const _Float16* __restrict__ qt,
                                                                const _Float16* __restrict__ enc, int Tq, int T,
-                                                               int NG, float* __restrict__ sbuf) {
+                                                               int NG, float* __restrict__ sbuf, int resq) {
   constexpr int CW = D / NW, KS = CW / 32, HP = HT * 16, ROW = NS * D;
   __shared__ __attribute__((aligned(16))) float red[NW][HT][16][20];
   const int g = blockIdx.x, r = blockIdx.y;
@@ -677,11 +685,18 @@
   const _Float16* E = enc + (size_t)(r / Tq) * T * ROW;
   half8 a[KS][NS];
   const int fc = f < T ? f : T - 1;
-#pragma unroll
-  for (int ks = 0; ks < KS; ++ks)
-#pragma unroll
-    for (int p = 0; p < NS; ++p)
-      a[ks][p] = *reinterpret_cast<const half8*>(E + (size_t)fc * ROW + p * D + c0 + ks * 32 + 8 * lq);
+  const half8* ap = reinterpret_cast<const half8*>(E + (size_t)fc * ROW + c0 + 8 * lq);
+  if (xattn_chunk_resident(g, resq)) {
+#pragma unroll
+    for (int ks = 0; ks < KS; ++ks)
+#pragma unroll
+      for (int p = 0; p < NS; ++p) a[ks][p] = ap[(p * D + ks * 32) / 8];
+  } else {
+#pragma unroll
+    for (int ks = 0; ks < KS; ++ks)
+#pragma unroll
+      for (int p = 0; p < NS; ++p) a[ks][p] = __builtin_nontemporal_load(&ap[(p * D + ks * 32) / 8]);
+  }
   if (f >= T) {
 #pragma unroll
     for (int ks = 0; ks < KS; ++ks)
@@ -732,7 +747,7 @@
 __global__ __launch_bounds__(256) void xattn_z_kernel(const _Float16* __restrict__ enc,
                                                       const float* __restrict__ sbuf, int Tq, int T, int H, int S,
                                                       int CH, int NG, float* __restrict__ zpart,
-                                                      float* __restrict__ mlpart) {
+                                                      float* __restrict__ mlpart, int resq) {
   constexpr int ROW = NS * D, ZR = 32, HP = HT * 16;
   constexpr int SMX = 512 / 256;
   __shared__ __attribute__((aligned(16))) _Float16 sp[kSmallMaxCH][NS][32][kTc];
@@ -751,11 +766,17 @@
       const_cast<_Float16*>(E + (size_t)ts * ROW), 0, nch > 0 ? (te - ts) * ROW * 2 : 0, 0x00020000);
   u32x4v ev[kSmallMaxCH][NS];
 #pragma unroll
-  for (int c = 0; c < kSmallMaxCH; ++c)
-#pragma unroll
-    for (int p = 0; p < NS; ++p)
-      ev[c][p] = __builtin_amdgcn_raw_buffer_load_b128(
-          rs, (uint32_t)((((c * kTc + (l >> 2)) * ROW) + p * D + cb + 8 * (l & 3)) * 2), 0, 0);
+  for (int c = 0; c < kSmallMaxCH; ++c) {
+    const uint32_t eo = (uint32_t)((((c * kTc + (l >> 2)) * ROW) + cb + 8 * (l & 3)) * 2);
+    if (xattn_chunk_resident(s * CH + c, resq)) {
+#pragma unroll
+      for (int p = 0; p < NS; ++p) ev[c][p] = __builtin_amdgcn_raw_buffer_load_b128(rs, eo + p * D * 2, 0, 0);
+    } else {
+#pragma unroll
+      for (int p = 0; p < NS; ++p)
+        ev[c][p] = __builtin_amdgcn_raw_buffer_load_b128(rs, eo + p * D * 2, 0, WA_XATTN_STREAM_AUX);
+    }
+  }
   float sv_all[kSmallMaxCH][SMX];
 #pragma unroll
   for (int c = 0; c < kSmallMaxCH; ++c)
@@ -846,13 +867,14 @@
 
 template <int D, int HT, int NS>
 void launch_small(int R, int Tq, int T, int H, const XattnPlan& p, const _Float16* qt, const _Float16* enc,
-                  float* z, float* ml, float* scratch, hipStream_t st) {
+                  float* z, float* ml, float* scratch, int resq, hipStream_t st) {
   constexpr int NW = (D / 8) % 32 == 0 ? 8 : 4;
   const int NG = p.splits * p.ch;
   float* sb = scratch;
-  hipLaunchKernelGGL((xattn_scores_kernel<D, HT, NS, NW>), dim3(NG, R), dim3(64 * NW), 0, st, qt, enc, Tq, T, NG, sb);
+  hipLaunchKernelGGL((xattn_scores_kernel<D, HT, NS, NW>), dim3(NG, R), dim3(64 * NW), 0, st, qt, enc, Tq, T, NG, sb,
+                     resq);
   hipLaunchKernelGGL((xattn_z_kernel<D, HT, NS>), dim3(p.splits, D / 128, R), dim3(256), 0, st, enc, sb, Tq, T, H,
-                     p.splits, p.ch, NG, z, ml);
+                     p.splits, p.ch, NG, z, ml, resq);
 }
 
 int xattn_small_rows() {
@@ -863,10 +885,14 @@
 
 template <int D, int HT, int NS>
 void launch_main(dim3 g, const _Float16* qt, const _Float16* enc, int Tq, int T, int H, int S, int CH, float* z,
-                 float* ml, int R, hipStream_t st) {
+                 float* ml, int R, int resq, hipStream_t st) {
   constexpr int NW = (D / 8) % 32 == 0 ? 8 : 4;
-  hipLaunchKernelGGL((xattn_main_kernel<D, HT, NS, NW, 1>), g, dim3(64 * NW), 0, st, qt, enc, Tq, T, H, S, CH, z, ml,
-                     R);
+  if (resq >= kXattnResDen)
+    hipLaunchKernelGGL((xattn_main_kernel<D, HT, NS, NW, 1, false>), g, dim3(64 * NW), 0, st, qt, enc, Tq, T, H, S,
+                       CH, z, ml, R, resq);
+  else
+    hipLaunchKernelGGL((xattn_main_kernel<D, HT, NS, NW, 1, true>), g, dim3(64 * NW), 0, st, qt, enc, Tq, T, H, S, CH,
+                       z, ml, R, resq);
 }
 
 #ifndef WA_XATTN_OUT_ROWS
@@ -914,6 +940,26 @@
   return p;
 }
 
+constexpr double kXattnFitMB = 268.4;
+constexpr double kXattnResidentMB = 172.0;
+XattnResidency xattn_residency(int live_clips, int T, int ns, int D, double budget_mb) {
+  const double live = (double)live_clips * T * ns * D * 2.0;
+  double fit = kXattnFitMB;
+  if (budget_mb < 0.0) {
+    budget_mb = kXattnResidentMB;
+    if (const char* e = getenv("WA_XATTN_RESIDENT_MB")) budget_mb = fit = std::max(0.0, atof(e));
+  } else {
+    fit = budget_mb;
+  }
+  XattnResidency r;
+  const double budget = std::min(budget_mb, 1e9) * 1e6;
+  if (live <= std::max(fit * 1e6, budget))
+    r.q = kXattnResDen;
+  else
+    r.q = std::max(0, std::min(kXattnResDen - 1, (int)std::floor(kXattnResDen * budget / live)));
+  return r;
+}
+
 size_t xattn_part_floats(int R, int H, int D, int T) {
   const XattnPlan p = xattn_plan(R, T);
   size_t n = (size_t)R * p.splits * H * ((size_t)D + 2) + (size_t)R * H * D;
@@ -954,10 +1000,11 @@
 
 hipError_t launch_xattn(const float* q, const uint8_t* wk, const uint8_t* wv, const uint32_t* wvp, const float* bv,
                         int wtype, const _Float16* enc, int B, int Tq, int T, int H, int D, _Float16* qt, float* part,
-                        _Float16* tiled, int ns, hipStream_t st, float* out32) {
+                        _Float16* tiled, int ns, XattnResidency res, hipStream_t st, float* out32) {
   const int R = B * Tq;
   const int HT = (H + 15) / 16, HP = HT * 16;
   if (D != H * 64 || D % 128 != 0 || D > kMaxD || H > 20 || !q) return hipErrorInvalidValue;
+  if (res.q < 0 || res.q > kXattnResDen) return hipErrorInvalidValue;
   if (wtype == kWtQ4 && !wvp) return hipErrorInvalidValue;
   const XattnPlan p = xattn_plan(R, T);
   float* z = part;
@@ -977,13 +1024,13 @@
   if (D == DD && HT == HH) {                                                               \
     if (small) {                                                                           \
       if (ns == 2)                                                                         \
-        launch_small<DD, HH, 2>(R, Tq, T, H, p, qt, enc, z, ml, scratch, st);              \
+        launch_small<DD, HH, 2>(R, Tq, T, H, p, qt, enc, z, ml, scratch, res.q, st);       \
       else                                                                                 \
-        launch_small<DD, HH, 1>(R, Tq, T, H, p, qt, enc, z, ml, scratch, st);              \
+        launch_small<DD, HH, 1>(R, Tq, T, H, p, qt, enc, z, ml, scratch, res.q, st);       \
     } else if (ns == 2)                                                                    \
-      launch_main<DD, HH, 2>(gm, qt, enc, Tq, T, H, p.splits, p.ch, z, ml, R, st);          \
+      launch_main<DD, HH, 2>(gm, qt, enc, Tq, T, H, p.splits, p.ch, z, ml, R, res.q, st);  \
     else                                                                                   \
-      launch_main<DD, HH, 1>(gm, qt, enc, Tq, T, H, p.splits, p.ch, z, ml, R, st);          \
+      launch_main<DD, HH, 1>(gm, qt, enc, Tq, T, H, p.splits, p.ch, z, ml, R, res.q, st);  \
   } else
   WA_XMAIN(1280, 2)
   WA_XMAIN(1024, 1)
diff --git a/whisper-burn_amd/whisper_amd/__init__.py b/whisper-burn_amd/whisper_amd/__init__.py
--- a/whisper-burn_amd/whisper_amd/__init__.py
+++ b/whisper-burn_amd/whisper_amd/__init__.py
@@ -68,6 +68,14 @@
         L.wa_log_mel.argtypes = [c_int, vp, c_int, c_i64, c_i64, c_int, vp, vp]
         L.wa_mel_filterbank.argtypes = [c_int, f32p, f32p]
         L.wa_xattn_check.argtypes = [c_int, vp, vp, vp, vp, c_int, vp, c_int, c_int, c_int, c_int, c_int, vp]
+        L.wa_xattn_resident_share.argtypes = [c_int, c_int, c_int, c_int, ctypes.c_double]
+        L.wa_xattn_resident_share.restype = c_int
+        L.wa_xattn_chunk_resident.argtypes = [c_int, c_int]
+        L.wa_xattn_chunk_resident.restype = c_int
+        L.wa_xattn_plan.argtypes = [c_int, ctypes.POINTER(c_int), ctypes.POINTER(c_int)]
+        L.wa_xattn_plan.restype = c_int
+        L.wa_decode_graph_key.argtypes = [vp, c_int]
+        L.wa_decode_graph_key.restype = ctypes.c_longlong
         L.wa_xattn_kv_check.argtypes = [c_int, vp, vp, vp, c_int, c_int, c_int, c_int, c_int, vp]
         L.wa_transcribe_trace.argtypes = [vp, vp, c_int, c_int, c_int, c_int, i32p, i32p, vp, c_int, vp, vp]
         L.wa_encoder_attention_check.argtypes = [c_int, vp, c_int, c_int, c_int, c_int, vp]
@@ -143,6 +151,29 @@
     check(lib().wa_xattn_check(dev, ptr(q), ptr(wk_raw), ptr(wv_raw), ptr(bv), weight_type, ptr(enc), B, Tq, T, H,
                                precision, ptr(out)))
     return out
+
+
+XATTN_SHARE_DEN = 64
+
+
+def xattn_resident_share(live_clips: int, T: int, planes: int, D: int, budget_mb: float = -1.0) -> int:
+    q = int(lib().wa_xattn_resident_share(live_clips, T, planes, D, budget_mb))
+    if q < 0:
+        raise ValueError("bad sizes")
+    return q
+
+
+def xattn_chunk_resident(chunk: int, share: int) -> bool:
+    r = int(lib().wa_xattn_chunk_resident(chunk, share))
+    if r < 0:
+        raise ValueError("bad chunk / share")
+    return bool(r)
+
+
+def xattn_plan(T: int) -> tuple[int, int]:
+    s, c = ctypes.c_int(), ctypes.c_int()
+    check(lib().wa_xattn_plan(T, ctypes.byref(s), ctypes.byref(c)))
+    return s.value, c.value
 
 
 def xattn_kv_check(q, k, v, Tq: int, precision: int = wq4.PREC_F16X2):
@@ -312,6 +343,9 @@
     def pipeline_pairs(self) -> int:
         return int(lib().wa_last_pipeline_pairs(self._h))
 
+    def decode_graph_key(self, group: int = 0) -> int:
+        return int(lib().wa_decode_graph_key(self._h, group))
+
     def transcribe_trace(self, mel, trace_ids: np.ndarray, lang_token: Optional[int] = 50259,
                          max_tokens: int = 224, eot_stop: bool = False):
         torch = _torch()
```

Measured after the change: 1129, median of 6. +4.1%, better.
